# TurakhiaLab/DIPPER

Measured on AMD Instinct MI355X. Metric: tips/sec FASTA->Newick at N=30000, higher is better.
Workload: dtype f64

## Files before the change

### dipper_amd/capi.py

```python
import ctypes as C
import os

import numpy as np

_HERE = os.path.dirname(os.path.abspath(__file__))
_LIB = None

SRC_MSA, SRC_MASH, SRC_MATRIX = 1, 2, 3
DIST_UNCORRECTED, DIST_JC = 1, 2
DIST_POISSON, DIST_KIMURA = 7, 8
DIST_TN93, DIST_LOGDET, DIST_PARALINEAR = 9, 10, 11

c_i32p = C.POINTER(C.c_int32)
c_i64p = C.POINTER(C.c_int64)
c_u64p = C.POINTER(C.c_uint64)
c_f64p = C.POINTER(C.c_double)


class DipperError(RuntimeError):
    def __init__(self, code, msg):
        super().__init__(f"dipper_hip error {code}: {msg}")
        self.code = code


def library_path():
    return os.environ.get("DPR_LIB") or os.path.join(_HERE, "libdipper_hip.so")


def load_library():
    global _LIB
    if _LIB is not None:
        return _LIB
    path = library_path()
    if not os.path.exists(path):
        raise FileNotFoundError(f"{path} not built: run `python -c 'import __graft_entry__ as g; g.build()'`")
    L = C.CDLL(path)
    L.dpr_last_error.restype = C.c_char_p
    L.dpr_abi_version.restype = C.c_int
    L.dpr_pack4.argtypes = [C.c_char_p, C.c_uint64, c_u64p]
    L.dpr_pack2.argtypes = [C.c_char_p, C.c_uint64, c_u64p]
    L.dpr_pack_aa.argtypes = [C.c_char_p, C.c_uint64, C.POINTER(C.c_uint8)]
    L.dpr_njr_owner.argtypes = [C.c_int64, C.c_int]
    L.dpr_njr_local_row.argtypes = [C.c_int64, C.c_int]
    L.dpr_njr_local_row.restype = C.c_int64
    L.dpr_njr_global_pos.argtypes = [C.c_int64, C.c_int, C.c_int]
    L.dpr_njr_global_pos.restype = C.c_int64
    L.dpr_njr_rows_cap.argtypes = [C.c_int64, C.c_int]
    L.dpr_njr_rows_cap.restype = C.c_int64
    L.dpr_shard_owner.argtypes = [C.c_int64, C.c_int]
    L.dpr_shard_local_row.argtypes = [C.c_int64, C.c_int]
    L.dpr_shard_local_row.restype = C.c_int64
    L.dpr_shard_rows.argtypes = [C.c_int64, C.c_int, C.c_int]
    L.dpr_shard_rows.restype = C.c_int64
    L.dpr_shard_global_row.argtypes = [C.c_int64, C.c_int, C.c_int]
    L.dpr_shard_global_row.restype = C.c_int64
    L.dpr_record_reduce.argtypes = [C.c_void_p, C.c_int]
    L.dpr_nj_key.argtypes = [C.c_int64, C.c_int64, C.c_int64]
    L.dpr_nj_key.restype = C.c_uint64
    L.dpr_create.argtypes = [C.POINTER(C.c_void_p), C.c_int]
    L.dpr_create_virtual.argtypes = [C.POINTER(C.c_void_p), C.c_int, C.c_int]
    L.dpr_destroy.argtypes = [C.c_void_p]
    L.dpr_device_name.argtypes = [C.c_void_p, C.c_char_p, C.c_int]
    L.dpr_comm_unique_id.argtypes = [C.c_void_p]
    L.dpr_comm_init.argtypes = [C.c_void_p, C.c_int, C.c_int, C.c_void_p]
    L.dpr_comm_selftest.argtypes = [C.c_void_p]
    L.dpr_comm_info.argtypes = [C.c_void_p, C.POINTER(C.c_int), C.POINTER(C.c_int)]
    L.dpr_comm_init_local.argtypes = [C.c_void_p, C.c_int, C.c_int]
    L.dpr_comm_init_shared.argtypes = [C.c_void_p, C.c_int, C.c_int, C.c_void_p, C.c_uint64, C.c_int]
    L.dpr_comm_stats.argtypes = [C.c_void_p, C.POINTER(C.c_int), C.POINTER(C.c_int64)]
    L.dpr_shared_abort.argtypes = [C.c_void_p]
    L.dpr_shared_failed.argtypes = [C.c_void_p]
    L.dpr_shared_barrier.argtypes = [C.c_void_p, C.c_int, C.POINTER(C.c_uint32), C.c_int]
    L.dpr_shared_gather.argtypes = [C.c_void_p, C.c_int, C.c_int, C.POINTER(C.c_uint32), C.c_int, C.c_void_p, C.c_void_p, C.c_int]
    L.dpr_peer_export.argtypes = [C.c_void_p, C.c_int64, C.c_void_p]
    L.dpr_peer_attach.argtypes = [C.c_void_p, C.c_void_p]
    L.dpr_ctx_set_nj_exchange.argtypes = [C.c_void_p, C.c_int]
    L.dpr_get_nj_exchange_info.argtypes = [C.c_void_p, C.POINTER(C.c_int), C.POINTER(C.c_int64), C.POINTER(C.c_int64), C.c_char_p, C.c_int]
    L.dpr_ctx_set_poll_limit_ms.argtypes = [C.c_void_p, C.c_int]
    L.dpr_ctx_set_nj_adaptive.argtypes = [C.c_void_p, C.c_int]
    L.dpr_get_nj_adaptive_stats.argtypes = [C.c_void_p, C.POINTER(C.c_int64), C.POINTER(C.c_int64)]
    L.dpr_scan_tune.argtypes = [C.c_int, C.c_int, C.c_int]
    L.dpr_set_nj_mode.argtypes = [C.c_int]
    L.dpr_set_nj_multi_plan.argtypes = [C.c_int]
    L.dpr_nj_is_unit_sharded.argtypes = [C.c_void_p]
    L.dpr_get_nj_multi_info.argtypes = [C.c_void_p, C.c_char_p, C.c_int]
    L.dpr_ctx_set_nj_mode.argtypes = [C.c_void_p, C.c_int]
    L.dpr_ctx_set_nj_multi_plan.argtypes = [C.c_void_p, C.c_int]
    L.dpr_ctx_set_nj_virtual_shards.argtypes = [C.c_void_p, C.c_int]
    L.dpr_ctx_set_nj_kernel_timing.argtypes = [C.c_void_p, C.c_int]
    L.dpr_ctx_set_nj_variant.argtypes = [C.c_void_p, C.c_int]
    L.dpr_get_nj_lambda.argtypes = [C.c_void_p, c_f64p, C.POINTER(C.c_int64)]
    L.dpr_nj_variant_host.argtypes = [C.c_int, c_f64p, C.c_int64, C.c_int64, c_i32p, c_i32p, c_f64p, c_f64p, c_f64p, c_f64p]
    L.dpr_nj_variant_host.restype = C.c_int64
    L.dpr_get_nj_kernel_timing.argtypes = [C.c_void_p, C.POINTER(C.c_int), c_f64p, C.POINTER(C.c_int64)]
    L.dpr_nj_kernel_name.argtypes = [C.c_int]
    L.dpr_nj_kernel_name.restype = C.c_char_p
    L.dpr_get_place_timing.argtypes = [C.c_void_p, c_f64p, c_f64p]
    L.dpr_get_place_overlap.argtypes = [C.c_void_p, C.POINTER(C.c_int), c_f64p]
    L.dpr_get_place_policy.argtypes = [C.c_void_p, C.POINTER(C.c_int64), C.POINTER(C.c_int64)]
    L.dpr_get_prune_stats.argtypes = [C.c_void_p, c_u64p, c_u64p]
    L.dpr_ctx_set_debug_fault.argtypes = [C.c_void_p, C.c_int64, C.c_int]
    L.dpr_get_nj_progress.argtypes = [C.c_void_p, C.POINTER(C.c_int64), C.POINTER(C.c_int64)]
    L.dpr_get_njp_shape.argtypes = [C.c_void_p, C.POINTER(C.c_int64), C.POINTER(C.c_int), C.POINTER(C.c_int), C.POINTER(C.c_int), C.POINTER(C.c_int)]
    L.dpr_bw_probe.argtypes = [C.c_void_p, C.c_int64, C.c_int, C.c_int, C.c_int, C.POINTER(C.c_float)]
    L.dpr_set_msa.argtypes = [C.c_void_p, c_u64p, C.c_int64, C.c_int64]
    L.dpr_set_msa_aa.argtypes = [C.c_void_p, C.POINTER(C.c_uint8), C.c_int64, C.c_int64]
    L.dpr_set_reads.argtypes = [C.c_void_p, c_u64p, c_u64p, c_u64p, C.c_int64]
    L.dpr_set_matrix_lower.argtypes = [C.c_void_p, c_f64p, C.c_int64]
    L.dpr_sketch.argtypes = [C.c_void_p, C.c_int, C.c_int, c_u64p]
    L.dpr_get_mash_index_info.argtypes = [C.c_void_p, c_i64p]
    L.dpr_dist_matrix.argtypes = [C.c_void_p, C.c_int, C.c_int, C.c_int]
    L.dpr_reserve_nj.argtypes = [C.c_void_p, C.c_int64]
    L.dpr_warm_graphs.argtypes = [C.c_void_p]
    L.dpr_nj_run.argtypes = [C.c_void_p, C.c_int64, c_i32p, c_i32p, c_f64p, c_f64p, c_f64p]
    L.dpr_nj_run.restype = C.c_int64
    L.dpr_argmin_once.argtypes = [C.c_void_p, C.c_int, c_i32p, c_i32p, c_f64p, C.POINTER(C.c_float)]
    L.dpr_n_active.argtypes = [C.c_void_p]
    L.dpr_n_active.restype = C.c_int64
    L.dpr_n_total.argtypes = [C.c_void_p]
    L.dpr_n_total.restype = C.c_int64
    L.dpr_get_matrix_row.argtypes = [C.c_void_p, C.c_int64, c_f64p]
    L.dpr_get_row_sums.argtypes = [C.c_void_p, c_f64p]
    L.dpr_get_msa_counts.argtypes = [C.c_void_p, C.c_int64, c_i32p, c_i32p]
    L.dpr_msa_dist_block.argtypes = [C.c_void_p, C.c_int64, C.c_int64, C.c_int64, C.c_int, C.c_int, c_f64p, C.c_int, C.POINTER(C.c_float)]
    L.dpr_get_kmer_hashes.argtypes = [C.c_void_p, C.c_int64, C.c_int, c_u64p, c_u64p, c_u64p]
    L.dpr_get_place_state.argtypes = [C.c_void_p, c_i32p, c_f64p, c_f64p]
    L.dpr_get_place_walks.argtypes = [C.c_void_p, c_i32p, C.POINTER(C.c_int64)]
    L.dpr_get_timing.argtypes = [C.c_void_p, c_f64p, c_f64p]
    L.dpr_place_run.argtypes = [C.c_void_p, C.c_int, C.c_int, C.c_int, C.c_int64, C.c_int64,
                                c_i32p, c_i32p, c_i32p, c_i32p, c_f64p]
    L.dpr_place_exact_run.argtypes = [C.c_void_p, C.c_int, C.c_int, C.c_int, C.c_int64,
                                      c_i32p, c_i32p, c_i32p, c_i32p, c_f64p]
    L.dpr_get_exact_state.argtypes = [C.c_void_p, c_i32p, c_i32p]
    L.dpr_dc_run.argtypes = [C.c_void_p, C.c_int, C.c_int, C.c_int, C.c_int64, C.c_int64, C.c_int,
                             c_i32p, c_i32p, c_i32p, c_i32p, c_f64p, c_i32p]
    L.dpr_place_fixed_set.argtypes = [C.c_void_p, C.c_int64, C.c_int64, c_i32p, c_i32p, c_i32p, c_i32p, c_f64p]
    L.dpr_place_fixed_run.argtypes = [C.c_void_p, C.c_int, C.c_int, C.c_int, c_i32p, c_f64p, c_f64p]
    L.dpr_ctx_set_place_fixed_batch.argtypes = [C.c_void_p, C.c_int64]
    L.dpr_get_place_fixed_timing.argtypes = [C.c_void_p, c_f64p, c_f64p]
    L.dpr_njp_unit_owner.argtypes = [C.c_int64, C.c_int64, C.c_int64, C.c_int]
    L.dpr_place_policy_run.argtypes = [C.c_int, C.c_int, C.c_int, C.c_int, C.c_int64, C.c_int64, C.c_int64, C.c_int64, c_f64p, c_f64p, C.c_int64, c_i32p]
    L.dpr_nj_plan_resolve.argtypes = [C.c_int, C.c_int, C.c_int, C.c_int, C.c_int, C.c_int, C.c_int64, C.c_uint64]
    L.dpr_dc_query_share.argtypes = [C.c_int64, C.c_int64, C.c_int, C.c_int, C.POINTER(C.c_int64), C.POINTER(C.c_int64)]
    L.dpr_dc_deal_clusters.argtypes = [C.POINTER(C.c_int64), C.c_int64, C.c_int, c_i32p]
    L.dpr_get_dc_stats.argtypes = [C.c_void_p, C.POINTER(C.c_int64), c_f64p]
    L.dpr_get_dc_table_stats.argtypes = [C.c_void_p, c_i64p]
    L.dpr_msa_resample.argtypes = [C.c_void_p, C.c_uint64, C.c_int64]
    L.dpr_get_msa_boot_weights.argtypes = [C.c_void_p, c_i32p]
    L.dpr_msa_boot_weights.argtypes = [C.c_uint64, C.c_int64, C.c_int64, c_i32p]
    L.dpr_get_msa_site_coverage.argtypes = [C.c_void_p, c_i32p]
    L.dpr_msa_filter_sites.argtypes = [C.c_void_p, C.c_int]
    L.dpr_msa_filter_sites.restype = C.c_int64
    L.dpr_split_support.argtypes = [C.c_int64, c_i32p, c_i32p, c_i32p, c_i32p, c_i32p]
    L.dpr_comm_sum_i32.argtypes = [C.c_void_p, c_i32p, C.c_int64]
    L.dpr_transfer_support.argtypes = [C.c_void_p, C.c_int64, c_i32p, c_i32p, c_i32p, c_i32p, c_i64p]
    _bme_out = [C.c_int, c_i32p, c_i32p, c_f64p, c_f64p, c_i64p]
    L.dpr_bme_nni.argtypes = [C.c_void_p, C.c_int64, c_i32p, c_i32p] + _bme_out
    L.dpr_bme_nni_host.argtypes = [c_f64p, C.c_int64, c_i32p, c_i32p] + _bme_out
    L.dpr_bme_eval_host.argtypes = [c_f64p, C.c_int64, c_i32p, C.c_int32, c_f64p, c_f64p, c_i32p, c_f64p]
    L.dpr_get_bme_timing.argtypes = [C.c_void_p, c_f64p, c_f64p]
    L.dpr_get_bme_stats.argtypes = [C.c_void_p, c_i64p]
    L.dpr_bme_spr.argtypes = [C.c_void_p, C.c_int64, c_i32p, c_i32p] + _bme_out
    L.dpr_bme_spr_host.argtypes = [c_f64p, C.c_int64, c_i32p, c_i32p] + _bme_out
    L.dpr_bme_spr_eval_host.argtypes = [c_f64p, C.c_int64, c_i32p, C.c_int32, c_f64p, c_i32p, c_i32p, c_f64p]
    L.dpr_bme_spr_gain_host.argtypes = [c_f64p, C.c_int64, c_i32p, C.c_int32, C.c_int64, C.c_int32, c_f64p, c_i32p]
    L.dpr_get_bme_spr_timing.argtypes = [C.c_void_p, c_f64p]
    L.dpr_get_bme_spr_stats.argtypes = [C.c_void_p, c_i64p]
    L.dpr_upgma_run.argtypes = [C.c_void_p, C.c_int, c_i32p, c_i32p, c_f64p]
    L.dpr_upgma_run.restype = C.c_int64
    L.dpr_upgma_host.argtypes = [c_f64p, C.c_int64, C.c_int, c_i32p, c_i32p, c_f64p]
    L.dpr_get_upgma_stats.argtypes = [C.c_void_p, c_i64p]
    L.dpr_get_upgma_timing.argtypes = [C.c_void_p, c_f64p]
    L.dpr_transfer_support_host.argtypes = [C.c_int64, c_i32p, c_i32p, c_i32p, c_i32p, c_i64p]
    L.dpr_transfer_taxa.argtypes = [C.c_void_p, C.c_int64, c_i32p, c_i32p, c_i32p, c_i32p, C.c_int, c_i64p, c_i64p, c_i64p]
    L.dpr_transfer_taxa_host.argtypes = [C.c_int64, c_i32p, c_i32p, c_i32p, c_i32p, C.c_int, c_i64p, c_i64p, c_i64p]
    L.dpr_ctx_set_tbe_lds.argtypes = [C.c_void_p, C.c_int64]
    L.dpr_comm_sum_i64.argtypes = [C.c_void_p, c_i64p, C.c_int64]
    _LIB = L
    return L


DC_EXACT_LAST = 1
COMM_SHARED_BYTES = 65536
TRANSPORT_AUTO, TRANSPORT_RCCL, TRANSPORT_IPC = 0, 1, 2


class SharedRegion:

    def __init__(self, name, create=False):
        import mmap
        self.path = os.path.join("/dev/shm", name)
        if create:
            with open(self.path, "wb") as f:
                f.write(b"\0" * COMM_SHARED_BYTES)
        self._f = open(self.path, "r+b")
        self._m = mmap.mmap(self._f.fileno(), COMM_SHARED_BYTES)
        self._buf = (C.c_char * COMM_SHARED_BYTES).from_buffer(self._m)
        self.address = C.addressof(self._buf)
        self.size = COMM_SHARED_BYTES

    def abort(self):
        load_library().dpr_shared_abort(self.address)

    def failed(self):
        return bool(load_library().dpr_shared_failed(self.address))

    def barrier(self, world, sense, timeout_ms=10000):
        L = load_library()
        _chk(L, L.dpr_shared_barrier(self.address, world, C.byref(sense), timeout_ms))

    def gather(self, rank, world, sense, mine: bytes, timeout_ms=10000):
        L = load_library()
        out = (C.c_char * (len(mine) * world))()
        _chk(L, L.dpr_shared_gather(self.address, rank, world, C.byref(sense), timeout_ms, mine, out, len(mine)))
        return [bytes(out[r * len(mine):(r + 1) * len(mine)]) for r in range(world)]

    def unlink(self):
        try:
            os.unlink(self.path)
        except OSError:
            pass


def dc_virtual_ranks(w):
    return (w & 0xff) << 8


def set_nj_virtual_shards(w):
    L = load_library()
    _chk(L, L.dpr_set_nj_virtual_shards(w))


def set_nj_mode(mode):
    L = load_library()
    _chk(L, L.dpr_set_nj_mode(mode))


def set_nj_multi_plan(plan):
    L = load_library()
    _chk(L, L.dpr_set_nj_multi_plan(plan))


def _chk(L, rc):
    if rc < 0:
        raise DipperError(rc, (L.dpr_last_error() or b"").decode())
    return rc


(NJ_PLAN_SINGLE_STREAM, NJ_PLAN_SINGLE_PRUNED, NJ_PLAN_BIONJ, NJ_PLAN_ROWS_STREAM, NJ_PLAN_REPLICAS, NJ_PLAN_UNIT_SHARDED,
 NJ_PLAN_ROWS_PRUNED) = range(7)


def nj_plan_resolve(world, virtual_ranks, variant, pruned, multi_plan, virtual_shards, n, total_bytes):
    L = load_library()
    return _chk(L, L.dpr_nj_plan_resolve(world, int(virtual_ranks), variant, int(pruned), multi_plan, virtual_shards, n, total_bytes))


def place_policy_run(source, world, window_transport, no_overlap, multi_min, first, last, batch_rows, tree_ms, dist_alone_ms):
    L = load_library()
    tree = np.ascontiguousarray(tree_ms, dtype=np.float64)
    dist = np.ascontiguousarray(dist_alone_ms, dtype=np.float64)
    assert tree.shape == dist.shape and tree.ndim == 1
    beside = np.zeros(max(len(tree), 1), dtype=np.int32)
    _chk(L, L.dpr_place_policy_run(source, world, int(window_transport), int(no_overlap), multi_min, first, last, batch_rows,
                                   _p(tree, c_f64p), _p(dist, c_f64p), len(tree), _p(beside, c_i32p)))
    return [bool(b) for b in beside[:len(tree)]]


def _p(a, t):
    return a.ctypes.data_as(t)


def pack4(seq: bytes):
    L = load_library()
    out = np.zeros((len(seq) + 15) // 16, dtype=np.uint64)
    _chk(L, L.dpr_pack4(seq, len(seq), _p(out, c_u64p)))
    return out


def pack2(seq: bytes):
    L = load_library()
    out = np.zeros((len(seq) + 31) // 32, dtype=np.uint64)
    _chk(L, L.dpr_pack2(seq, len(seq), _p(out, c_u64p)))
    return out


def pack_aa(seq: bytes):
    L = load_library()
    out = np.zeros(len(seq), dtype=np.uint8)
    _chk(L, L.dpr_pack_aa(seq, len(seq), _p(out, C.POINTER(C.c_uint8))))
    return out


def pack_aa_many(seqs):
    Ls = len(seqs[0])
    out = np.full((len(seqs), Ls), 255, dtype=np.uint8)
    for i, s in enumerate(seqs):
        c = pack_aa(s)
        out[i, : min(Ls, len(c))] = c[:Ls]
    return out


def msa_boot_weights(seed, replicate, L):
    lib = load_library()
    out = np.zeros(L, dtype=np.int32)
    _chk(lib, lib.dpr_msa_boot_weights(seed, replicate, L, _p(out, c_i32p)))
    return out


def split_support(n, main_x, main_y, rep_x, rep_y, counts=None):
    lib = load_library()
    k = max(n - 2, 1)
    mx, my, rx, ry = (np.ascontiguousarray(np.asarray(a, dtype=np.int32)[: n - 2]) for a in (main_x, main_y, rep_x, rep_y))
    if counts is None:
        counts = np.zeros(k, dtype=np.int32)
    assert counts.dtype == np.int32 and counts.flags.c_contiguous and len(counts) >= n - 2
    _chk(lib, lib.dpr_split_support(n, _p(mx, c_i32p), _p(my, c_i32p), _p(rx, c_i32p), _p(ry, c_i32p), _p(counts, c_i32p)))
    return counts


def _tbe_args(n, main_x, main_y, rep_x, rep_y, phi_sum):
    logs = [np.ascontiguousarray(np.asarray(a, dtype=np.int32)[: n - 2]) for a in (main_x, main_y, rep_x, rep_y)]
    if phi_sum is None:
        phi_sum = np.zeros(max(n - 2, 1), dtype=np.int64)
    assert phi_sum.dtype == np.int64 and phi_sum.flags.c_contiguous and len(phi_sum) >= n - 2
    return logs, phi_sum


def transfer_support_host(n, main_x, main_y, rep_x, rep_y, phi_sum=None):
    lib = load_library()
    (mx, my, rx, ry), phi_sum = _tbe_args(n, main_x, main_y, rep_x, rep_y, phi_sum)
    _chk(lib, lib.dpr_transfer_support_host(n, _p(mx, c_i32p), _p(my, c_i32p), _p(rx, c_i32p), _p(ry, c_i32p), _p(phi_sum, c_i64p)))
    return phi_sum


def _taxa_args(n, moved, pairs):
    if moved is None:
        moved = np.zeros(max(n, 1), dtype=np.int64)
    if pairs is None:
        pairs = np.zeros(1, dtype=np.int64)
    assert moved.dtype == np.int64 and moved.flags.c_contiguous and len(moved) >= n
    assert pairs.dtype == np.int64 and pairs.flags.c_contiguous and len(pairs) >= 1
    return moved, pairs


def transfer_taxa_host(n, main_x, main_y, rep_x, rep_y, cutoff_permille=300, phi_sum=None, moved=None, pairs=None):
    lib = load_library()
    (mx, my, rx, ry), phi_sum = _tbe_args(n, main_x, main_y, rep_x, rep_y, phi_sum)
    moved, pairs = _taxa_args(n, moved, pairs)
    _chk(lib, lib.dpr_transfer_taxa_host(n, _p(mx, c_i32p), _p(my, c_i32p), _p(rx, c_i32p), _p(ry, c_i32p), cutoff_permille,
                                         _p(phi_sum, c_i64p), _p(moved, c_i64p), _p(pairs, c_i64p)))
    return phi_sum, moved, pairs


def _bme_args(n, merge_x, merge_y, max_rounds, nstats=4):
    mx, my = (np.ascontiguousarray(np.asarray(a, dtype=np.int32)[: max(n - 2, 0)]) for a in (merge_x, merge_y))
    assert len(mx) == len(my) == n - 2
    out = dict(kids=np.zeros(2 * max(n - 2, 1), dtype=np.int32), top=np.zeros(1, dtype=np.int32), len=np.zeros(2 * n - 2, dtype=np.float64),
               L_rounds=np.zeros(max_rounds + 1, dtype=np.float64), stats=np.zeros(nstats, dtype=np.int64))
    ptrs = (_p(mx, c_i32p), _p(my, c_i32p), max_rounds, _p(out["kids"], c_i32p), _p(out["top"], c_i32p), _p(out["len"], c_f64p),
            _p(out["L_rounds"], c_f64p), _p(out["stats"], c_i64p))
    return (mx, my), out, ptrs


def _bme_result(n, out):
    rounds, moves, fallbacks, cands0 = (int(v) for v in out["stats"][:4])
    more = dict(long_moves=int(out["stats"][4]), max_k=int(out["stats"][5])) if len(out["stats"]) == 6 else {}
    return dict(**more, kids=out["kids"][: 2 * (n - 2)].reshape(n - 2, 2), top=int(out["top"][0]), len=out["len"], L_rounds=out["L_rounds"][: rounds + 1],
                rounds=rounds, moves=moves, fallbacks=fallbacks, candidates0=cands0)


def bme_nni_host(D, merge_x, merge_y, max_rounds):
    lib = load_library()
    D = np.asarray(D, dtype=np.float64)
    n = D.shape[0]
    rows = np.ascontiguousarray(np.concatenate([D[i, :i] for i in range(n)])) if n > 1 else np.zeros(1)
    keep, out, ptrs = _bme_args(n, merge_x, merge_y, max_rounds)
    _chk(lib, lib.dpr_bme_nni_host(_p(rows, c_f64p), n, *ptrs))
    return _bme_result(n, out)


def bme_eval_host(D, kids, top):
    lib = load_library()
    D = np.asarray(D, dtype=np.float64)
    n = D.shape[0]
    rows = np.ascontiguousarray(np.concatenate([D[i, :i] for i in range(n)]))
    kids = np.ascontiguousarray(np.asarray(kids, dtype=np.int32).reshape(-1))
    assert len(kids) == 2 * (n - 2)
    ln, gain, move = np.zeros(2 * n - 2), np.zeros(2 * n - 2), np.zeros(2 * n - 2, dtype=np.int32)
    L = C.c_double(0.0)
    _chk(lib, lib.dpr_bme_eval_host(_p(rows, c_f64p), n, _p(kids, c_i32p), int(top), _p(ln, c_f64p), _p(gain, c_f64p), _p(move, c_i32p), C.byref(L)))
    return dict(len=ln, gain=gain, move=move, L=L.value)


def _lower_rows(D):
    D = np.asarray(D, dtype=np.float64)
    n = D.shape[0]
    return n, (np.ascontiguousarray(np.concatenate([D[i, :i] for i in range(n)])) if n > 1 else np.zeros(1))


def bme_spr_host(D, merge_x, merge_y, max_rounds):
    lib = load_library()
    n, rows = _lower_rows(D)
    keep, out, ptrs = _bme_args(n, merge_x, merge_y, max_rounds, 6)
    _chk(lib, lib.dpr_bme_spr_host(_p(rows, c_f64p), n, *ptrs))
    return _bme_result(n, out)


def bme_spr_eval_host(D, kids, top):
    lib = load_library()
    n, rows = _lower_rows(D)
    kids = np.ascontiguousarray(np.asarray(kids, dtype=np.int32).reshape(-1))
    assert len(kids) == 2 * (n - 2)
    m2 = 2 * (2 * n - 2)
    gain, w, k = np.zeros(m2), np.zeros(m2, dtype=np.int32), np.zeros(m2, dtype=np.int32)
    L = C.c_double(0.0)
    _chk(lib, lib.dpr_bme_spr_eval_host(_p(rows, c_f64p), n, _p(kids, c_i32p), int(top), _p(gain, c_f64p), _p(w, c_i32p), _p(k, c_i32p), C.byref(L)))
    return dict(gain=gain, w=w, k=k, L=L.value)


def bme_spr_gain_host(D, kids, top, d, w):
    lib = load_library()
    n, rows = _lower_rows(D)
    kids = np.ascontiguousarray(np.asarray(kids, dtype=np.int32).reshape(-1))
    assert len(kids) == 2 * (n - 2)
    g, k = C.c_double(0.0), C.c_int32(0)
    _chk(lib, lib.dpr_bme_spr_gain_host(_p(rows, c_f64p), n, _p(kids, c_i32p), int(top), int(d), int(w), C.byref(g), C.byref(k)))
    return g.value, k.value


NJ_VARIANT_NJ, NJ_VARIANT_BIONJ = 0, 1


def upgma_host(D, linkage=0):
    lib = load_library()
    n, rows = _lower_rows(D)
    cnt = max(n - 1, 1)
    mx, my, h = np.zeros(cnt, dtype=np.int32), np.zeros(cnt, dtype=np.int32), np.zeros(cnt, dtype=np.float64)
    _chk(lib, lib.dpr_upgma_host(_p(rows, c_f64p), n, int(linkage), _p(mx, c_i32p), _p(my, c_i32p), _p(h, c_f64p)))
    return dict(merge_x=mx[: n - 1], merge_y=my[: n - 1], height=h[: n - 1])


def nj_variant_host(variant, D, max_iters=-1):
    lib = load_library()
    D = np.asarray(D, dtype=np.float64)
    n = D.shape[0]
    rows = np.ascontiguousarray(np.concatenate([D[i, :i] for i in range(n)])) if n > 1 else np.zeros(1)
    k = max(n - 2, 1)
    mx = np.zeros(k, dtype=np.int32)
    my = np.zeros(k, dtype=np.int32)
    bx = np.zeros(k, dtype=np.float64)
    by = np.zeros(k, dtype=np.float64)
    lam = np.full(k, 0.5, dtype=np.float64)
    last = C.c_double(0.0)
    done = _chk(lib, lib.dpr_nj_variant_host(variant, _p(rows, c_f64p), n, max_iters, _p(mx, c_i32p), _p(my, c_i32p), _p(bx, c_f64p),
                                             _p(by, c_f64p), C.byref(last), _p(lam, c_f64p)))
    return dict(iters=done, merge_x=mx[:done], merge_y=my[:done], bl_x=bx[:done], bl_y=by[:done], last_d=last.value, lam=lam[:done])


def pack4_many(seqs):
    Ls = len(seqs[0])
    W = (Ls + 15) // 16
    out = np.zeros((len(seqs), W), dtype=np.uint64)
    for i, s in enumerate(seqs):
        w = pack4(s)
        out[i, : min(W, len(w))] = w[:W]
    return out


class Dipper:

    def __init__(self, device=0, virtual_world=0):
        self.L = load_library()
        h = C.c_void_p()
        if virtual_world:
            _chk(self.L, self.L.dpr_create_virtual(C.byref(h), device, virtual_world))
        else:
            _chk(self.L, self.L.dpr_create(C.byref(h), device))
        self.h = h

    def close(self):
        if self.h:
            self.L.dpr_destroy(self.h)
            self.h = None

    def __del__(self):
        try:
            self.close()
        except Exception:
            pass

    def device_name(self):
        buf = C.create_string_buffer(256)
        _chk(self.L, self.L.dpr_device_name(self.h, buf, 256))
        return buf.value.decode()

    def comm_unique_id(self):
        buf = (C.c_char * 128)()
        _chk(self.L, self.L.dpr_comm_unique_id(buf))
        return bytes(buf)

    def comm_init(self, rank, world, uid: bytes):
        buf = (C.c_char * 128).from_buffer_copy(uid) if uid else None
        _chk(self.L, self.L.dpr_comm_init(self.h, rank, world, buf))

    def comm_selftest(self):
        _chk(self.L, self.L.dpr_comm_selftest(self.h))

    def comm_init_local(self, rank, world):
        _chk(self.L, self.L.dpr_comm_init_local(self.h, rank, world))

    def comm_init_shared(self, rank, world, region, transport=0):
        self._region = region
        _chk(self.L, self.L.dpr_comm_init_shared(self.h, rank, world, region.address, region.size, transport))

    def comm_stats(self):
        t = C.c_int()
        n = C.c_int64()
        _chk(self.L, self.L.dpr_comm_stats(self.h, C.byref(t), C.byref(n)))
        return ["none", "rccl", "ipc", "local"][t.value], int(n.value)

    def peer_export(self, n_tips):
        buf = (C.c_char * 192)()
        _chk(self.L, self.L.dpr_peer_export(self.h, n_tips, buf))
        return bytes(buf)

    def peer_attach(self, blobs):
        data = b"".join(blobs)
        buf = (C.c_char * len(data)).from_buffer_copy(data)
        _chk(self.L, self.L.dpr_peer_attach(self.h, buf))

    def set_nj_exchange(self, plan):
        _chk(self.L, self.L.dpr_ctx_set_nj_exchange(self.h, plan))

    def nj_exchange_info(self):
        p = C.c_int()
        nl = C.c_int64()
        nc = C.c_int64()
        note = C.create_string_buffer(256)
        _chk(self.L, self.L.dpr_get_nj_exchange_info(self.h, C.byref(p), C.byref(nl), C.byref(nc), note, 256))
        return {"plan": {0: "legacy", 1: "peer", 2: "mailbox"}.get(p.value, str(p.value)), "launches": int(nl.value),
                "collectives": int(nc.value), "note": note.value.decode()}

    def set_nj_adaptive(self, on):
        _chk(self.L, self.L.dpr_ctx_set_nj_adaptive(self.h, on))

    def nj_adaptive_stats(self):
        a = C.c_int64()
        b = C.c_int64()
        _chk(self.L, self.L.dpr_get_nj_adaptive_stats(self.h, C.byref(a), C.byref(b)))
        return int(a.value), int(b.value)

    def set_debug_fault(self, iteration, rank):
        _chk(self.L, self.L.dpr_ctx_set_debug_fault(self.h, iteration, rank))

    def set_poll_limit_ms(self, ms):
        _chk(self.L, self.L.dpr_ctx_set_poll_limit_ms(self.h, ms))

    def comm_info(self):
        r = C.c_int()
        n = C.c_int()
        _chk(self.L, self.L.dpr_comm_info(self.h, C.byref(r), C.byref(n)))
        return r.value, n.value

    def set_msa(self, packed4, L):
        p = np.ascontiguousarray(packed4, dtype=np.uint64)
        _chk(self.L, self.L.dpr_set_msa(self.h, _p(p, c_u64p), p.shape[0], L))
        self._msa_sites = int(L)

    def set_msa_aa(self, codes):
        p = np.ascontiguousarray(codes, dtype=np.uint8)
        assert p.ndim == 2
        _chk(self.L, self.L.dpr_set_msa_aa(self.h, _p(p, C.POINTER(C.c_uint8)), p.shape[0], p.shape[1]))
        self._msa_sites = int(p.shape[1])

    def set_matrix_lower(self, rows, n):
        r = np.ascontiguousarray(rows, dtype=np.float64)
        assert r.size == n * (n - 1) // 2
        _chk(self.L, self.L.dpr_set_matrix_lower(self.h, _p(r, c_f64p), n))

    def set_matrix_full(self, D):
        D = np.asarray(D, dtype=np.float64)
        n = D.shape[0]
        rows = np.concatenate([D[i, :i] for i in range(n)]) if n > 1 else np.zeros(0)
        self.set_matrix_lower(rows, n)

    def set_reads(self, seqs):
        words = [pack2(s) for s in seqs]
        lens = np.array([len(s) for s in seqs], dtype=np.uint64)
        nw = np.array([len(w) for w in words], dtype=np.uint64)
        off = np.zeros(len(seqs), dtype=np.uint64)
        off[1:] = np.cumsum(nw)[:-1]
        flat = np.concatenate(words) if len(words) else np.zeros(0, np.uint64)
        if flat.size == 0:
            flat = np.zeros(1, np.uint64)
        self._reads = (np.ascontiguousarray(flat), off, lens)
        _chk(self.L, self.L.dpr_set_reads(self.h, _p(self._reads[0], c_u64p), _p(off, c_u64p), _p(lens, c_u64p), len(seqs)))

    def set_reads_packed(self, flat, off, lens):
        flat = np.ascontiguousarray(flat, dtype=np.uint64)
        off = np.ascontiguousarray(off, dtype=np.uint64)
        lens = np.ascontiguousarray(lens, dtype=np.uint64)
        self._reads = (flat, off, lens)
        _chk(self.L, self.L.dpr_set_reads(self.h, _p(flat, c_u64p), _p(off, c_u64p), _p(lens, c_u64p), len(lens)))

    def sketch(self, k=15, S=1000, fetch=True):
        n = len(self._reads[2])
        out = np.zeros((n, S), dtype=np.uint64) if fetch else None
        _chk(self.L, self.L.dpr_sketch(self.h, k, S, _p(out, c_u64p) if fetch else None))
        return out

    def mash_index_info(self):
        info = np.zeros(8, dtype=np.int64)
        _chk(self.L, self.L.dpr_get_mash_index_info(self.h, _p(info, c_i64p)))
        names = ("built", "chunk_tips", "chunks", "distinct", "dense", "dense_min", "max_sketch", "beside_task_bound")
        return {nm: int(v) for nm, v in zip(names, info)}

    def kmer_hashes(self, seq, k):
        _, off, lens = self._reads
        nk = max(int(lens[seq]) - k + 1, 0)
        out = np.zeros(max(nk, 1), dtype=np.uint64)
        _chk(self.L, self.L.dpr_get_kmer_hashes(self.h, seq, k, _p(off, c_u64p), _p(lens, c_u64p), _p(out, c_u64p)))
        return out[:nk]

    def place_run(self, source, n, first=2, dist_type=1, k=15, state=None):
        st = state or dict(head=np.full(2 * n, -1, np.int32), e=np.full(8 * n, -1, np.int32),
                           nxt=np.full(8 * n, -1, np.int32), belong=np.full(8 * n, -1, np.int32),
                           len=np.full(8 * n, 2.0, np.float64))
        _chk(self.L, self.L.dpr_place_run(self.h, source, dist_type, k, first, n, _p(st["head"], c_i32p),
                                          _p(st["e"], c_i32p), _p(st["nxt"], c_i32p), _p(st["belong"], c_i32p),
                                          _p(st["len"], c_f64p)))
        cid = np.zeros(40 * n, np.int32)
        cdis = np.zeros(40 * n, np.float64)
        trace = np.zeros(3 * n, np.float64)
        _chk(self.L, self.L.dpr_get_place_state(self.h, _p(cid, c_i32p), _p(cdis, c_f64p), _p(trace, c_f64p)))
        st.update(cid=cid, cdis=cdis, trace=trace.reshape(n, 3))
        return st

    def place_exact_run(self, source, n, dist_type=1, k=15):
        st = dict(head=np.full(2 * n, -1, np.int32), e=np.full(8 * n, -1, np.int32),
                  nxt=np.full(8 * n, -1, np.int32), belong=np.full(8 * n, -1, np.int32),
                  len=np.full(8 * n, 2.0, np.float64))
        _chk(self.L, self.L.dpr_place_exact_run(self.h, source, dist_type, k, n, _p(st["head"], c_i32p),
                                                _p(st["e"], c_i32p), _p(st["nxt"], c_i32p),
                                                _p(st["belong"], c_i32p), _p(st["len"], c_f64p)))
        rev = np.zeros(8 * n, np.int32)
        dep = np.zeros(2 * n, np.int32)
        trace = np.zeros(3 * n, np.float64)
        _chk(self.L, self.L.dpr_get_exact_state(self.h, _p(rev, c_i32p), _p(dep, c_i32p)))
        _chk(self.L, self.L.dpr_get_place_state(self.h, None, None, _p(trace, c_f64p)))
        st.update(rev=rev, dep=dep, trace=trace.reshape(n, 3))
        return st

    def dc_run(self, source, n, backbone, dist_type=1, k=15, flags=0):
        st = dict(head=np.full(2 * n, -1, np.int32), e=np.full(8 * n, -1, np.int32),
                  nxt=np.full(8 * n, -1, np.int32), belong=np.full(8 * n, -1, np.int32),
                  len=np.full(8 * n, 2.0, np.float64))
        cl = np.full(n, -1, np.int32)
        _chk(self.L, self.L.dpr_dc_run(self.h, source, dist_type, k, n, backbone, flags, _p(st["head"], c_i32p),
                                       _p(st["e"], c_i32p), _p(st["nxt"], c_i32p), _p(st["belong"], c_i32p),
                                       _p(st["len"], c_f64p), _p(cl, c_i32p)))
        cid = np.zeros(40 * n, np.int32)
        cdis = np.zeros(40 * n, np.float64)
        trace = np.zeros(3 * n, np.float64)
        _chk(self.L, self.L.dpr_get_place_state(self.h, _p(cid, c_i32p), _p(cdis, c_f64p), _p(trace, c_f64p)))
        counts = np.zeros(5, np.int64)
        ms = np.zeros(3, np.float64)
        _chk(self.L, self.L.dpr_get_dc_stats(self.h, counts.ctypes.data_as(C.POINTER(C.c_int64)), _p(ms, c_f64p)))
        st.update(cid=cid, cdis=cdis, trace=trace.reshape(n, 3), cluster_id=cl,
                  stats=dict(clusters=int(counts[0]), max_cluster=int(counts[1]), pairs=int(counts[2]),
                             groups=int(counts[3]), jobs=int(counts[4]), backbone_ms=float(ms[0]),
                             assign_ms=float(ms[1]), cluster_ms=float(ms[2])))
        return st

    def dc_table_stats(self):
        out = np.zeros(4, dtype=np.int64)
        _chk(self.L, self.L.dpr_get_dc_table_stats(self.h, _p(out, c_i64p)))
        return {nm: int(v) for nm, v in zip(("entries", "chunks", "max_entries", "max_leaves"), out)}

    def place_fixed_set(self, m, n, state):
        st = {k: np.ascontiguousarray(state[k], dtype=np.float64 if k == "len" else np.int32) for k in ("head", "e", "nxt", "belong", "len")}
        assert st["head"].size >= 2 * n and all(st[k].size >= 8 * n for k in ("e", "nxt", "belong", "len"))
        _chk(self.L, self.L.dpr_place_fixed_set(self.h, m, n, _p(st["head"], c_i32p), _p(st["e"], c_i32p), _p(st["nxt"], c_i32p),
                                                _p(st["belong"], c_i32p), _p(st["len"], c_f64p)))
        self._pfix_nq = n - m

    def place_fixed_run(self, source, dist_type=1, k=15):
        nq = max(getattr(self, "_pfix_nq", 1), 1)
        slot = np.full(nq, -2, np.int32)
        frac = np.zeros(nq, np.float64)
        add = np.zeros(nq, np.float64)
        _chk(self.L, self.L.dpr_place_fixed_run(self.h, source, dist_type, k, _p(slot, c_i32p), _p(frac, c_f64p), _p(add, c_f64p)))
        return slot, frac, add

    def set_place_fixed_batch(self, queries):
        _chk(self.L, self.L.dpr_ctx_set_place_fixed_batch(self.h, queries))

    def place_fixed_timing(self):
        a = C.c_double()
        b = C.c_double()
        _chk(self.L, self.L.dpr_get_place_fixed_timing(self.h, C.byref(a), C.byref(b)))
        return a.value, b.value

    def warm_graphs(self):
# ... 274 lines not shown
```

### dipper_amd/csrc/ctx_nj.hip

```cpp
#include "ctx_internal.hpp"

#include <chrono>
#include <cstdio>

namespace dpr {
static int g_nj_mode = -1;
static int g_nj_vshards = 1;
static int g_nj_multi_plan = -1;
constexpr int64_t kNjShardTips = 65536;
static int nj_multi_plan()
{
    if (g_nj_multi_plan < 0) {
        const char* e = std::getenv("DPR_NJ_MULTI");
        g_nj_multi_plan = (e && std::strcmp(e, "shard") == 0) ? 1 : (e && std::strcmp(e, "solo") == 0) ? 2 : (e && std::strcmp(e, "rows") == 0) ? 3 : 0;
    }
    return g_nj_multi_plan;
}

bool want_pruned(const dpr_ctx* c)
{
    if (c->nj_mode >= 0) return c->nj_mode == 1;
    if (g_nj_mode < 0) {
        const char* e = std::getenv("DPR_NJ_MODE");
        g_nj_mode = (e && std::strcmp(e, "stream") == 0) ? 0 : 1;
// ... 101 lines not shown
    if (!c->plan.rows_dealt()) return DPR_OK;
    if (int rc = njs_setup(c, njr)) return rc;
    if (njr && c->plan.exchange == kNjsLegacy) {
        set_error("dpr_dist_matrix: the row-sharded pruned NJ needs the peers' buffers mapped on every rank (" + c->nj_exchange_note + "); use DPR_NJ_MODE=stream");
        return DPR_ERR_STATE;
    }
    return DPR_OK;
}
static int dist_fill(dpr_ctx* c, int source, int dist_type, int64_t n)
{
    for (auto& b : c->nj) {
        if (source == DPR_SRC_MSA) {
            if (int rc = msa_dist_rows(c->msa, b, dist_type, c->stream)) return rc;
        } else if (source == DPR_SRC_MASH) {
            if (b.world > 1) {
                if (int rc = mash_dist_matrix_sharded(c->mash, b.rank, b.world, b.rows_local, b.D, b.ld, c->stream)) return rc;
            } else {
                for (int64_t r0 = 0; r0 < b.rows_local; r0 += 32768) {
                    const int64_t nr = b.rows_local - r0 < 32768 ? b.rows_local - r0 : 32768;
                    if (int rc = mash_dist_rows(c->mash, r0, nr, b.rank, b.world, true, n, b.D + r0 * b.ld, b.ld, c->stream)) return rc;
                }
            }
        } else {
            if (int rc = nj_expand_lower(b, c->packed_lower, c->stream)) return rc;
        }
        if (c->plan.kind == DPR_NJ_PLAN_BIONJ)
            if (int rc = nj_bionj_init(b, c->stream)) return rc;
    }
    return DPR_OK;
}
static int dist_row_sums(dpr_ctx* c)
{
    const bool dealt = c->plan.rows_dealt(), windows = dealt && c->plan.exchange != kNjsLegacy;
    for (auto& b : c->nj)
        if (int rc = nj_init_sums(b, c->stream, !dealt ? nullptr : windows ? reinterpret_cast<double*>(b.peer.win + b.peer.lay.off_slice) : b.slice)) return rc;
    if (dealt)
        if (int rc = windows ? njs_barrier(c) : exchange(c, EX_U)) return rc;
    for (auto& b : c->nj) {
        if (dealt)
            if (int rc = windows ? njs_launch_unpack_u(b, c->stream) : nj_launch_unpack_u(b, c->stream)) return rc;
        if (int rc = nj_prepare(b, c->stream)) return rc;
    }
    return DPR_OK;
}
static int dist_build_njr(dpr_ctx* c)
{
    int rplan = c->nj_exchange == 2 ? kNjrMailbox : c->nj_exchange == 1 ? kNjrCollective : (c->local_comm ? kNjrMailbox : kNjrCollective);
    if (c->nj_exchange < 0 && !c->local_comm)
        if (const char* e = std::getenv("DPR_NJ_EXCHANGE")) rplan = std::strcmp(e, "mailbox") == 0 ? kNjrMailbox : kNjrCollective;
    if (rplan == kNjrCollective && c->vworld == 0 && !comm_real(c)) { set_error("dpr_dist_matrix: the collective plan of the row-sharded pruned NJ needs a transport between the ranks (RCCL, or dpr_comm_init_shared)"); return DPR_ERR_STATE; }
    for (auto& b : c->nj) {
        b.rs.world = c->world; b.rs.rank = b.rank; b.rs.plan = rplan;
        b.rs.win_off = b.peer.lay.off_njr;
        b.rs.gather = njr_gather_cb; b.rs.cb_ctx = c;
        b.rs.barrier = (c->vworld == 0 && (c->comm || (c->shm && rplan == kNjrCollective))) ? njr_barrier_cb : nullptr;
        b.rs.launches = 0; b.rs.collectives = 0;
    }
    std::vector<NjBuffers*> ranks = njr_ranks(c);
    if (int rc = njr_build(ranks, c->stream)) return rc;
    c->nj_exchange_note = std::string("row-sharded pruned NJ (njr.hip), exchange plan ") + (rplan == kNjrMailbox ? "mailbox" : "collective");
    return DPR_OK;
}
static void njp_set_shards(dpr_ctx* c, int kind)
{
    NjPruned& q = c->nj[0].pr;
    if (kind == DPR_NJ_PLAN_UNIT_SHARDED) { q.sh_world = c->world; q.sh_rank = c->rank; q.sh_virtual = false; q.gather = njp_gather_cb; q.gather_ctx = c; }
    else if (ctx_vshards(c) > 1) { q.sh_world = ctx_vshards(c); q.sh_rank = 0; q.sh_virtual = true; }
}
static int dist_build_njp(dpr_ctx* c)
{
    NjPruned& q = c->nj[0].pr;
    njp_set_shards(c, c->plan.kind);
    if (c->nj_adaptive >= 0) q.adaptive = c->nj_adaptive;
    if (int rc = njp_build(c->nj[0], c->stream)) return rc;
    if (c->nj_adaptive >= 0) q.adaptive = c->nj_adaptive;
    return DPR_OK;
}
static bool plan_is_njp(int kind) { return kind == DPR_NJ_PLAN_SINGLE_PRUNED || kind == DPR_NJ_PLAN_REPLICAS || kind == DPR_NJ_PLAN_UNIT_SHARDED; }

}

using namespace dpr;

__global__ void dpr_warm_kernel(int x);

extern "C" {

int dpr_dist_matrix(dpr_ctx* c, int source, int dist_type, int k)
{
    if (!c) { set_error("dpr_dist_matrix: null ctx"); return DPR_ERR_ARG; }
    DPR_HIP(hipSetDevice(c->device));
    if (c->world > 1 && c->vworld == 0 && !c->comm && !c->local_comm && !c->shm) { set_error("dpr_dist_matrix: dpr_comm_init was not called"); return DPR_ERR_STATE; }
    int64_t n = 0;
    if (source == DPR_SRC_MSA) {
        if (!c->msa.planes) { set_error("dpr_dist_matrix: call dpr_set_msa first"); return DPR_ERR_STATE; }
        n = c->msa.n;
    } else if (source == DPR_SRC_MATRIX) {
        if (!c->packed_lower) { set_error("dpr_dist_matrix: call dpr_set_matrix_lower first"); return DPR_ERR_STATE; }
        n = c->n_input;
    } else if (source == DPR_SRC_MASH) {
        if (!c->mash.sketches) { set_error("dpr_dist_matrix: call dpr_set_reads and dpr_sketch first"); return DPR_ERR_STATE; }
        if (k != c->mash.k) { set_error("dpr_dist_matrix: k differs from the sketch k"); return DPR_ERR_ARG; }
        n = c->mash.n;
    } else {
        set_error("dpr_dist_matrix: source not available");
        return DPR_ERR_ARG;
    }
    const int kind = ctx_nj_plan(c, n, "dpr_dist_matrix");
    if (kind < 0) return kind;
    c->have_matrix = 0;
    c->plan = NjPlan{ kind, kNjsLegacy };
    c->nj_exchange_note.clear();
    if (int rc = dist_alloc(c, n)) return rc;
    DPR_HIP(hipEventRecord(c->ev[0], c->stream));
    if (int rc = dist_fill(c, source, dist_type, n)) return rc;
    if (int rc = dist_row_sums(c)) return rc;
    if (int rc = kind == DPR_NJ_PLAN_ROWS_PRUNED ? dist_build_njr(c) : plan_is_njp(kind) ? dist_build_njp(c) : DPR_OK) return rc;
    DPR_HIP(hipEventRecord(c->ev[1], c->stream));
    DPR_HIP(hipStreamSynchronize(c->stream));
    float ms = 0;
    DPR_HIP(hipEventElapsedTime(&ms, c->ev[0], c->ev[1]));
    c->dist_ms = ms;
    c->have_matrix = 1;
    return DPR_OK;
}

int dpr_reserve_nj(dpr_ctx* c, int64_t n)
{
    if (!c || n < 2 || n >= (1 << 24)) { set_error("dpr_reserve_nj: bad argument"); return DPR_ERR_ARG; }
    DPR_HIP(hipSetDevice(c->device));
    const int kind = ctx_nj_plan(c, n, "dpr_reserve_nj");
    if (kind < 0) return kind;
    if (kind != DPR_NJ_PLAN_SINGLE_STREAM && kind != DPR_NJ_PLAN_SINGLE_PRUNED && kind != DPR_NJ_PLAN_BIONJ) return DPR_OK;
    c->have_matrix = 0;
    if (int rc = nj_alloc(c->nj[0], n, 0, 1, c->stream, 0, kind == DPR_NJ_PLAN_BIONJ)) return rc;
    if (kind == DPR_NJ_PLAN_SINGLE_PRUNED) {
        njp_set_shards(c, kind);
        if (int rc = njp_arena(c->nj[0].pr, n, c->stream)) return rc;
    }
    DPR_HIP(hipStreamSynchronize(c->stream));
    return DPR_OK;
}

int dpr_warm_graphs(dpr_ctx* c)
{
    if (!c) { set_error("dpr_warm_graphs: null ctx"); return DPR_ERR_ARG; }
    DPR_HIP(hipSetDevice(c->device));
    const bool tlog = log_level("cli") > 0;
    const auto t0 = std::chrono::steady_clock::now();
    auto lap = [&](const char* what) {
        if (tlog) std::fprintf(stderr, "  dpr_warm_graphs: %s at %.1f ms\n", what, std::chrono::duration<double, std::milli>(std::chrono::steady_clock::now() - t0).count());
    };
    hipStream_t st = c->stream;
    if (hipStreamBeginCapture(st, hipStreamCaptureModeThreadLocal) == hipSuccess) {
        hipLaunchKernelGGL(dpr_warm_kernel, dim3(1), dim3(64), 0, st, 0);
        ScopedGraph g;
        ScopedGraphExec ge;
        if (hipStreamEndCapture(st, g.put()) == hipSuccess && g) {
            if (hipGraphInstantiate(ge.put(), g, nullptr, nullptr, 0) == hipSuccess && ge) {
                lap("first hipGraphInstantiate");
                (void)hipGraphLaunch(ge, st);
                (void)hipStreamSynchronize(st);
                lap("graph replayed");
            }
        }
    }
    {
        DevBuf<char> d;
        constexpr size_t kWarmBytes = 512 << 10;
        if (d.alloc(kWarmBytes) == hipSuccess) {
            std::vector<char> h(kWarmBytes);
            (void)hipMemsetAsync(d, 0, kWarmBytes, st);
            (void)hipStreamSynchronize(st);
            (void)hipMemcpyAsync(h.data(), d, kWarmBytes, hipMemcpyDeviceToHost, st);
            (void)hipStreamSynchronize(st);
            (void)hipMemcpyAsync(d, h.data(), kWarmBytes, hipMemcpyHostToDevice, st);
            (void)hipStreamSynchronize(st);
        }
    }
    lap("staged copies both ways");
    (void)hipGetLastError();
    return DPR_OK;
}

}
namespace dpr {
int fetch_state(dpr_ctx* c, NjState* st)
{
    DPR_HIP(hipMemcpyAsync(st, c->nj[0].st, sizeof(NjState), hipMemcpyDeviceToHost, c->stream));
    DPR_HIP(hipStreamSynchronize(c->stream));
    return DPR_OK;
}
}
extern "C" {

int64_t dpr_nj_run(dpr_ctx* c, int64_t max_iters, int32_t* merge_x, int32_t* merge_y, double* bl_x,
                   double* bl_y, double* last_d)
{
    if (!c || !c->have_matrix) { set_error("dpr_nj_run: call dpr_dist_matrix first"); return DPR_ERR_STATE; }
    DPR_HIP(hipSetDevice(c->device));
    NjState st;
    if (int rc = fetch_state(c, &st)) return rc;
    int64_t todo = st.n - 2;
    if (todo < 0) todo = 0;
    if (max_iters >= 0 && max_iters < todo) todo = max_iters;
    const int64_t it0 = st.it;
    c->nj[0].kt = &c->nj_kt;
    if (c->nj_kt.stride > 0 && it0 == 0) { c->nj_kt.samples = 0; for (double& v : c->nj_kt.us_sum) v = 0; }
    c->nj_launches = 0; c->nj_collectives = 0;
    DPR_HIP(hipEventRecord(c->ev[2], c->stream));
    if (c->plan.kind == DPR_NJ_PLAN_ROWS_PRUNED) {
        std::vector<NjBuffers*> ranks = njr_ranks(c);
        c->nj[0].rs.launches = 0; c->nj[0].rs.collectives = 0;
        if (int rc = njr_run(ranks, it0, todo, c->stream)) return rc;
        c->nj_launches = c->nj[0].rs.launches; c->nj_collectives = c->nj[0].rs.collectives;
    } else if (plan_is_njp(c->plan.kind)) {
        if (int rc = njp_run(c->nj[0], it0, todo, c->stream)) return rc;
    } else {
        for (int64_t k = 0; k < todo; ++k)
            if (int rc = nj_iteration(c, st.n - k, it0 + k)) return rc;
    }
    DPR_HIP(hipEventRecord(c->ev[3], c->stream));
    if (c->plan.one_exchange_loop()) {
        if (int rc = njs_barrier(c)) return rc;
        for (auto& b : c->nj)
            if (int rc = njs_launch_finish(b, st.n - todo, it0 + todo, c->njs_pending, c->stream)) return rc;
        c->njs_pending = false;
        if (int rc = njs_barrier(c)) return rc;
    } else {
        for (auto& b : c->nj)
            if (!b.pr.active)
                if (int rc = nj_launch_finish(b, st.n - todo, it0 + todo, c->stream)) return rc;
    }
    if (int rc = fetch_state(c, &st)) return rc;
    float ms = 0;
    DPR_HIP(hipEventElapsedTime(&ms, c->ev[2], c->ev[3]));
    c->nj_ms = ms;
    if (!c->nj_kt.ev.empty()) {
        NjKernelTiming& kt = c->nj_kt;
        const size_t grp = (size_t)kt.nk + 1;
        for (size_t g0 = 0; kt.nk > 0 && g0 + grp <= kt.ev.size(); g0 += grp) {
            for (int k = 0; k < kt.nk; ++k) {
                float us = 0;
                if (hipEventElapsedTime(&us, kt.ev[g0 + (size_t)k], kt.ev[g0 + (size_t)k + 1]) == hipSuccess) kt.us_sum[k] += (double)us * 1e3;
            }
            ++kt.samples;
        }
        for (hipEvent_t e : kt.ev) (void)hipEventDestroy(e);
        kt.ev.clear();
    }
    const int64_t done = st.it - it0;
    if (done > 0) {
        if (merge_x) DPR_HIP(hipMemcpy(merge_x, c->nj[0].log_x + it0, sizeof(int32_t) * (size_t)done, hipMemcpyDeviceToHost));
        if (merge_y) DPR_HIP(hipMemcpy(merge_y, c->nj[0].log_y + it0, sizeof(int32_t) * (size_t)done, hipMemcpyDeviceToHost));
        if (bl_x) DPR_HIP(hipMemcpy(bl_x, c->nj[0].log_bx + it0, sizeof(double) * (size_t)done, hipMemcpyDeviceToHost));
        if (bl_y) DPR_HIP(hipMemcpy(bl_y, c->nj[0].log_by + it0, sizeof(double) * (size_t)done, hipMemcpyDeviceToHost));
    }
    if (st.status == 3) {
        set_error("dpr_nj_run: the exchange between the ranks failed (a rank's record did not arrive within the poll limit, or the all-gather delivered a stale one)");
        return DPR_ERR_COMM;
    }
    if (st.status == 4) {
        char msg[320];
        std::snprintf(msg, sizeof msg, "dpr_nj_run: the ranks' replicated row sums differ after %lld iterations (rank %d: %a, rank %d: %a): a row pulled from its owner "
                      "was stale or torn -- the merge log up to here is not trustworthy; use the legacy exchange (dpr_ctx_set_nj_exchange(ctx, 0))",
                      (long long)st.it, (int)st.x, st.q, (int)st.y, st.d);
        set_error(msg);
        return DPR_ERR_COMM;
    }
    if (st.status == 5) {
        set_error("dpr_nj_run: internal: the test blocks of the post kernel did not see the producer blocks' tag within 2 ms (njp_post2_kernel; DPR_NJP_POST2=0 selects the fused kernel)");
        return DPR_ERR_HIP;
    }
    if (st.status != 0) {
        set_error("dpr_nj_run: no Q candidate below the reference's init value 10000 (undefined in the reference)");
        return DPR_ERR_NOCAND;
    }
    if (last_d && st.n == 2) {
        NjBuffers& b0 = c->nj[0];
        int32_t pos01[2] = { 0, 1 };
        if (b0.pr.in_positions()) DPR_HIP(hipMemcpy(pos01, b0.pr.pos_of_slot, sizeof(pos01), hipMemcpyDeviceToHost));
        const double* row1 = slot_row(c, 1, pos01[1], true);
        const bool by_record = c->plan.rows_dealt() && c->vworld == 0 && c->plan.exchange == kNjsLegacy;
        if (row1 && !by_record) {
            DPR_HIP(hipMemcpy(last_d, row1 + pos01[0], sizeof(double), hipMemcpyDeviceToHost));
        } else {
            NjRecord rec{ 0.0, 0ull, 0.0, 0ull };
            if (row1) DPR_HIP(hipMemcpy(&rec.d, row1 + pos01[0], sizeof(double), hipMemcpyDeviceToHost));
            DPR_HIP(hipMemcpy(b0.recs + c->rank, &rec, sizeof(NjRecord), hipMemcpyHostToDevice));
            if (int rc = exchange(c, EX_RECS)) return rc;
            DPR_HIP(hipStreamSynchronize(c->stream));
            DPR_HIP(hipMemcpy(&rec, b0.recs + 0, sizeof(NjRecord), hipMemcpyDeviceToHost));
            *last_d = rec.d;
        }
    }
    return done;
}

int dpr_argmin_once(dpr_ctx* c, int reps, int32_t* out_i, int32_t* out_j, double* out_q, float* out_ms)
{
    if (!c || !c->have_matrix) { set_error("dpr_argmin_once: call dpr_dist_matrix first"); return DPR_ERR_STATE; }
    DPR_HIP(hipSetDevice(c->device));
    if (reps < 1) reps = 1;
    NjState st0;
    if (int rc = fetch_state(c, &st0)) return rc;
    auto probe = [&](NjBuffers& b) -> int {
        return b.pr.in_positions() ? nj_launch_scan(b, true, b.pr.P, 0, c->stream) : nj_launch_scan(b, true, st0.n, st0.it, c->stream);
    };
    for (auto& b : c->nj)
        if (int rc = probe(b)) return rc;
    DPR_HIP(hipEventRecord(c->ev[2], c->stream));
    for (int r = 0; r < reps; ++r)
        for (auto& b : c->nj)
            if (int rc = probe(b)) return rc;
    DPR_HIP(hipEventRecord(c->ev[3], c->stream));
    for (auto& b : c->nj)
        if (int rc = nj_launch_select_local(b, nj_scan_grid(), c->stream)) return rc;
    if (int rc = exchange(c, EX_RECS)) return rc;
    const int ew = c->plan.whole_matrix() ? 1 : c->world;
    std::vector<NjRecord> recs((size_t)ew);
    DPR_HIP(hipMemcpyAsync(recs.data(), c->nj[0].recs, sizeof(NjRecord) * (size_t)ew, hipMemcpyDeviceToHost, c->stream));
    DPR_HIP(hipStreamSynchronize(c->stream));
    float ms = 0;
    DPR_HIP(hipEventElapsedTime(&ms, c->ev[2], c->ev[3]));
    if (out_ms) *out_ms = ms / (float)reps;
    const int w = dpr_record_reduce(recs.data(), ew);
    if (w < 0 || !(recs[(size_t)w].q < 10000.0)) { set_error("dpr_argmin_once: no Q candidate below 10000"); return DPR_ERR_NOCAND; }
    const NjRecord& rec = recs[(size_t)w];
    if (out_i) *out_i = (int32_t)(rec.key & 0xFFFFFFull);
    if (out_j) *out_j = (int32_t)((rec.key >> 24) & 0xFFFFFFull);
    if (out_q) *out_q = rec.q;
    return DPR_OK;
}

int dpr_nj_plan_resolve(int world, int virtual_ranks, int variant, int pruned, int multi_plan, int virtual_shards, int64_t n, uint64_t total_bytes)
{
    if (world < 1 || variant < 0 || variant > 1 || multi_plan < 0 || multi_plan > 3 || virtual_shards < 1 || n < 2) { set_error("dpr_nj_plan_resolve: bad argument"); return DPR_ERR_ARG; }
    if (variant == 1) {
        if (!virtual_ranks && virtual_shards == 1) return DPR_NJ_PLAN_BIONJ;
        set_error("BIONJ runs the single-rank streaming plan: not on a context of virtual ranks or with virtual shards (dpr_set_nj_virtual_shards > 1)");
        return DPR_ERR_ARG;
    }
    if (!pruned || n < 3) return world > 1 ? DPR_NJ_PLAN_ROWS_STREAM : DPR_NJ_PLAN_SINGLE_STREAM;
    if (world == 1) return DPR_NJ_PLAN_SINGLE_PRUNED;
    if (multi_plan == 3) return DPR_NJ_PLAN_ROWS_PRUNED;
    if (virtual_ranks) return DPR_NJ_PLAN_ROWS_STREAM;
    if (multi_plan == 0 && 2.0 * 8.0 * (double)n * (double)n > 0.85 * (double)total_bytes) return DPR_NJ_PLAN_ROWS_PRUNED;
    return multi_plan == 1 || (multi_plan == 0 && n >= kNjShardTips) ? DPR_NJ_PLAN_UNIT_SHARDED : DPR_NJ_PLAN_REPLICAS;
}

int dpr_njp_unit_owner(int64_t strip, int64_t group, int64_t P, int world) { return njp_unit_owner(strip, group, P, world); }

int dpr_set_nj_virtual_shards(int w)
{
    if (w < 1 || w > 64) { set_error("dpr_set_nj_virtual_shards: 1 <= w <= 64"); return DPR_ERR_ARG; }
    g_nj_vshards = w;
    return DPR_OK;
}

int dpr_set_nj_multi_plan(int plan)
{
    if (plan < 0 || plan > 3) { set_error("dpr_set_nj_multi_plan: 0 auto, 1 unit-sharded, 2 single-GPU plan on every rank, 3 row-sharded pruned"); return DPR_ERR_ARG; }
    g_nj_multi_plan = plan;
    return DPR_OK;
}
int dpr_nj_is_unit_sharded(dpr_ctx* c) { return c && c->plan.kind == DPR_NJ_PLAN_UNIT_SHARDED ? 1 : 0; }
int dpr_get_nj_multi_info(dpr_ctx* c, char* buf, int cap)
{
    if (!c || !buf || cap <= 0) { set_error("dpr_get_nj_multi_info: bad argument"); return DPR_ERR_ARG; }
    static const char* const ex[] = { "legacy (two all-gathers per iteration)", "peer (one all-gather, rows pulled)", "mailbox (no collective)" };
    std::string s = "single rank";
    switch (c->plan.kind) {
    case DPR_NJ_PLAN_BIONJ: if (c->world > 1) s = "BIONJ, streaming, every rank its own copy"; break;
    case DPR_NJ_PLAN_ROWS_PRUNED: s = c->nj_exchange_note; break;
    case DPR_NJ_PLAN_UNIT_SHARDED: s = "pruned, matrix replicated, unit tests and scans sharded (one all-gather of block records per iteration)"; break;
    case DPR_NJ_PLAN_REPLICAS: s = "pruned, every rank runs the single-GPU plan on its own copy of the matrix (replicas)"; break;
    case DPR_NJ_PLAN_ROWS_STREAM: s = std::string("streaming, rows sharded block-cyclically, exchange ") + ex[c->plan.exchange >= 0 && c->plan.exchange <= 2 ? c->plan.exchange : 0]; break;
    }
    std::snprintf(buf, (size_t)cap, "%s", s.c_str());
    return DPR_OK;
}

int dpr_ctx_set_nj_mode(dpr_ctx* c, int mode)
{
    if (!c || mode < -1 || mode > 1) { set_error("dpr_ctx_set_nj_mode: mode must be -1, 0 or 1"); return DPR_ERR_ARG; }
    c->nj_mode = mode;
    return DPR_OK;
}
int dpr_ctx_set_nj_multi_plan(dpr_ctx* c, int plan)
{
    if (!c || plan < -1 || plan > 3) { set_error("dpr_ctx_set_nj_multi_plan: -1 default, 0 auto, 1 unit-sharded, 2 single-GPU plan on every rank, 3 row-sharded pruned"); return DPR_ERR_ARG; }
    c->nj_multi_plan = plan;
    return DPR_OK;
}
int dpr_ctx_set_nj_variant(dpr_ctx* c, int variant)
{
    if (!c || variant < 0 || variant > 1) { set_error("dpr_ctx_set_nj_variant: variant must be 0 (NJ) or 1 (BIONJ)"); return DPR_ERR_ARG; }
    c->nj_variant = variant;
    return DPR_OK;
}
int dpr_get_nj_lambda(dpr_ctx* c, double* out, int64_t* count)
{
    if (!c || !count) { set_error("dpr_get_nj_lambda: null argument"); return DPR_ERR_ARG; }
    if (!c->have_matrix || c->plan.kind != DPR_NJ_PLAN_BIONJ || !c->nj[0].log_lam) { set_error("dpr_get_nj_lambda: no BIONJ matrix (dpr_ctx_set_nj_variant(ctx, 1), then dpr_dist_matrix)"); return DPR_ERR_STATE; }
    DPR_HIP(hipSetDevice(c->device));
    NjState st;
    if (int rc = fetch_state(c, &st)) return rc;
    *count = st.it;
    if (out && st.it > 0) DPR_HIP(hipMemcpy(out, c->nj[0].log_lam, sizeof(double) * (size_t)st.it, hipMemcpyDeviceToHost));
    return DPR_OK;
}
int dpr_ctx_set_nj_kernel_timing(dpr_ctx* c, int stride)
{
    if (!c || stride < 0) { set_error("dpr_ctx_set_nj_kernel_timing: stride >= 0"); return DPR_ERR_ARG; }
    c->nj_kt.stride = stride;
    return DPR_OK;
}
int dpr_get_nj_kernel_timing(dpr_ctx* c, int* kernels, double* us_avg, int64_t* samples)
{
    if (!c) { set_error("dpr_get_nj_kernel_timing: null ctx"); return DPR_ERR_ARG; }
    if (kernels) *kernels = c->nj_kt.nk;
    if (samples) *samples = c->nj_kt.samples;
    if (us_avg) for (int k = 0; k < kNjKernelsMax; ++k) us_avg[k] = c->nj_kt.samples > 0 ? c->nj_kt.us_sum[k] / (double)c->nj_kt.samples : 0.0;
    return DPR_OK;
}
const char* dpr_nj_kernel_name(int idx) { return njp_kernel_name(idx); }
int dpr_get_nj_phase_stamps(uint64_t* out) { return njp_phase_stamps((unsigned long long*)out); }
int dpr_get_njp_list(dpr_ctx* c, int32_t* out, int64_t cap, int64_t* count, int64_t* positions, double* ur, int64_t ur_cap)
{
    if (!c || !out || !count || !positions) { set_error("dpr_get_njp_list: null argument"); return DPR_ERR_ARG; }
    DPR_HIP(hipSetDevice(c->device));
    return njp_debug_list(c->nj[0], out, cap, count, positions, ur, ur_cap);
}

int dpr_ctx_set_nj_virtual_shards(dpr_ctx* c, int w)
{
    if (!c || w < -1 || w == 0 || w > 64) { set_error("dpr_ctx_set_nj_virtual_shards: -1 or 1 <= w <= 64"); return DPR_ERR_ARG; }
    c->nj_vshards = w;
    return DPR_OK;
}

int dpr_set_nj_mode(int mode)
{
    if (mode != 0 && mode != 1) { set_error("dpr_set_nj_mode: mode must be 0 or 1"); return DPR_ERR_ARG; }
    g_nj_mode = mode;
    return DPR_OK;
}

int dpr_ctx_set_nj_adaptive(dpr_ctx* c, int on)
{
    if (!c || on < -1 || on > 1) { set_error("dpr_ctx_set_nj_adaptive: -1, 0 or 1"); return DPR_ERR_ARG; }
    c->nj_adaptive = on;
    return DPR_OK;
}
int dpr_get_nj_adaptive_stats(dpr_ctx* c, int64_t* stream_iterations, int64_t* stream_epochs)
{
    if (!c || !c->have_matrix || !c->nj[0].pr.active) { set_error("dpr_get_nj_adaptive_stats: pruned path not active"); return DPR_ERR_STATE; }
    if (stream_iterations) *stream_iterations = c->nj[0].pr.stream_iterations;
    if (stream_epochs) *stream_epochs = c->nj[0].pr.stream_epochs;
    return DPR_OK;
}

int dpr_get_prune_stats(dpr_ctx* c, uint64_t* units_scanned, uint64_t* units_per_full_scan)
{
    if (!c || !c->have_matrix || !c->nj[0].pr.active) { set_error("dpr_get_prune_stats: pruned path not active"); return DPR_ERR_STATE; }
    NjState st;
    if (int rc = fetch_state(c, &st)) return rc;
    if (units_scanned) *units_scanned = st.units_scanned;
    if (units_per_full_scan) *units_per_full_scan = (uint64_t)c->nj[0].pr.utot0;
    return DPR_OK;
}


int dpr_get_nj_progress(dpr_ctx* c, int64_t* iterations_done, int64_t* active)
{
    if (!c || !c->have_matrix) { set_error("dpr_get_nj_progress: call dpr_dist_matrix first"); return DPR_ERR_STATE; }
    DPR_HIP(hipSetDevice(c->device));
    NjState st;
    if (int rc = fetch_state(c, &st)) return rc;
    if (iterations_done) *iterations_done = st.it;
    if (active) *active = st.n;
    return DPR_OK;
}

}
namespace {
double host_tree256(double* c)
{
    for (int s = 128; s > 0; s >>= 1)
        for (int t = 0; t < s; ++t) c[t] = c[t] + c[t + s];
    return c[0];
}
double host_fold(const double* part, int64_t nchunk)
{
    double p[256];
    for (int t = 0; t < 256; ++t) {
        double acc = 0.0;
        for (int64_t c = t; c < nchunk; c += 256) acc += part[c];
        p[t] = acc;
    }
    return host_tree256(p);
}
}
extern "C" {

int64_t dpr_nj_variant_host(int variant, const double* lower_rows, int64_t N, int64_t max_iters, int32_t* merge_x, int32_t* merge_y,
                            double* bl_x, double* bl_y, double* last_d, double* lambda)
{
    if ((variant != 0 && variant != 1) || N < 2 || N >= (1 << 24) || (N > 2 && (!lower_rows || !merge_x || !merge_y || !bl_x || !bl_y))) {
        set_error("dpr_nj_variant_host: bad argument");
        return DPR_ERR_ARG;
    }
    const bool bionj = variant == 1;
    const int64_t ld = N;
    std::vector<double> D((size_t)(N * ld), 0.0), V, U((size_t)N), Ur((size_t)N), part((size_t)((N + 255) / 256 + 1));
    for (int64_t i = 0; i < N; ++i)
        for (int64_t j = 0; j < i; ++j) D[(size_t)(i * ld + j)] = D[(size_t)(j * ld + i)] = lower_rows[i * (i - 1) / 2 + j];
    if (bionj) V = D;
    for (int64_t i = 0; i < N; ++i) {
        double c[256];
        for (int t = 0; t < 256; ++t) {
            double acc = 0.0;
            for (int64_t j = t; j < N; j += 256)
                if (j != i) acc += D[(size_t)(i * ld + j)];
            c[t] = acc;
        }
        U[(size_t)i] = host_tree256(c);
    }
    int64_t it = 0;
    for (; it < N - 2; ++it) {
        if (max_iters >= 0 && it >= max_iters) break;
        const int64_t n = N - it, last = n - 1, nchunk = (n + 255) / 256;
        const double r = (double)(n - 2);
        for (int64_t i = 0; i < n; ++i) Ur[(size_t)i] = U[(size_t)i] / r;
        double bq = 10000.0;
        uint64_t bk = ~0ull;
        for (int64_t a = 1; a < n; ++a) {
            const double* row = D.data() + a * ld;
            const double ua = Ur[(size_t)a];
            for (int64_t c = 0; c < a; ++c) {
                const double dv = row[c], uc = Ur[(size_t)c];
                const double q1 = (dv - ua) - uc, q2 = (dv - uc) - ua;
                if (q1 <= bq) { const uint64_t k = dpr_nj_key(a, c, n); if (q1 < bq || k < bk) { bq = q1; bk = k; } }
                if (q2 <= bq) { const uint64_t k = dpr_nj_key(c, a, n); if (q2 < bq || k < bk) { bq = q2; bk = k; } }
            }
        }
        if (bk == ~0ull || !(bq < 10000.0)) break;
        const int64_t ki = (int64_t)(bk & 0xFFFFFFull), kj = (int64_t)((bk >> 24) & 0xFFFFFFull);
        const int64_t x = ki < kj ? ki : kj, y = ki < kj ? kj : ki;
        const double d = D[(size_t)(y * ld + x)];
        const double bx0 = (d + U[(size_t)x] / r - U[(size_t)y] / r) * 0.5, by0 = d - bx0;
        double blX = bx0, blY = by0;
        if (blX < 0) { blY += blX; blX = 0; }
        if (blY < 0) { blX += blY; blY = 0; }
        merge_x[it] = (int32_t)x; merge_y[it] = (int32_t)y; bl_x[it] = blX; bl_y[it] = blY;
        double lam = 0.5, vxy = 0.0;
        if (bionj) {
            vxy = V[(size_t)(y * ld + x)];
            for (int64_t c = 0; c < nchunk; ++c) {
                double v[256];
                for (int t = 0; t < 256; ++t) {
                    const int64_t k = c * 256 + t;
                    v[t] = (k < n && k != x && k != y) ? V[(size_t)(y * ld + k)] - V[(size_t)(x * ld + k)] : 0.0;
                }
                part[(size_t)c] = host_tree256(v);
            }
            const double ssum = host_fold(part.data(), nchunk);
            lam = 0.5 + ssum / (2.0 * r * vxy);
            if (vxy == 0.0 || lam != lam) lam = 0.5;
            else if (lam < 0.0) lam = 0.0;
            else if (lam > 1.0) lam = 1.0;
            if (lambda) lambda[it] = lam;
        }
        for (int64_t c = 0; c < nchunk; ++c) {
            double v[256];
            for (int t = 0; t < 256; ++t) {
                const int64_t i = c * 256 + t;
                double val = 0.0;
                if (i < n && i != x && i != y) {
                    const double dxi = D[(size_t)(x * ld + i)], dyi = D[(size_t)(y * ld + i)];
                    double vnew = 0.0;
                    if (bionj) {
                        const double vxi = V[(size_t)(x * ld + i)], vyi = V[(size_t)(y * ld + i)];
                        const double a = dxi - bx0, b = dyi - by0;
                        val = b + lam * (a - b);
                        vnew = vyi + lam * (vxi - vyi) - (lam * (1.0 - lam)) * vxy;
                    } else {
                        val = (dxi + dyi - d) * 0.5;
                    }
                    if (i != last) {
                        const double far = D[(size_t)(last * ld + i)];
                        U[(size_t)i] = U[(size_t)i] + (-dxi - dyi + val);
                        D[(size_t)(x * ld + i)] = val; D[(size_t)(i * ld + x)] = val;
                        D[(size_t)(y * ld + i)] = far; D[(size_t)(i * ld + y)] = far;
                        if (bionj) {
                            const double vfar = V[(size_t)(last * ld + i)];
                            V[(size_t)(x * ld + i)] = vnew; V[(size_t)(i * ld + x)] = vnew;
                            V[(size_t)(y * ld + i)] = vfar; V[(size_t)(i * ld + y)] = vfar;
                        }
                    } else {
                        U[(size_t)y] = U[(size_t)last] + (-dxi - dyi + val);
                        D[(size_t)(x * ld + y)] = val; D[(size_t)(y * ld + x)] = val;
                        if (bionj) { V[(size_t)(x * ld + y)] = vnew; V[(size_t)(y * ld + x)] = vnew; }
                    }
                }
                v[t] = val;
            }
            part[(size_t)c] = host_tree256(v);
        }
        U[(size_t)x] = host_fold(part.data(), nchunk);
    }
    if (it == N - 2 && last_d) *last_d = D[(size_t)(1 * ld + 0)];
// ... 11 lines not shown
```

### dipper_amd/csrc/dpr_internal.hpp

```cpp
#pragma once
#include <hip/hip_runtime.h>
#include <stdint.h>
#include <string>
#include <vector>

#include "../../include/dipper_hip.h"
#include "hip_scope.hpp"

namespace dpr {

constexpr int kRowBlock = DPR_ROW_BLOCK;
constexpr int kTileCols = 512;
constexpr int kScanBlocks = 8192;
constexpr int kThreads = 256;

void set_error(const std::string& msg);
int log_level(const char* category);
int hip_fail(hipError_t e, const char* what);
#define DPR_HIP(call)                                            \
    do {                                                         \
        hipError_t e__ = (call);                                 \
        if (e__ != hipSuccess) return dpr::hip_fail(e__, #call); \
    } while (0)

__host__ __device__ inline int shard_owner(int64_t row, int world)
{
    return (int)((row / kRowBlock) % world);
}
__host__ __device__ inline int64_t shard_local_row(int64_t row, int world)
{
    return (row / kRowBlock / world) * kRowBlock + row % kRowBlock;
}
__host__ __device__ inline int64_t shard_global_row(int64_t local, int rank, int world)
{
    return ((local / kRowBlock) * world + rank) * kRowBlock + local % kRowBlock;
}
__host__ __device__ inline int64_t shard_rows(int64_t n, int rank, int world)
{
    int64_t nblk = n / kRowBlock, rem = n % kRowBlock;
    int64_t full = nblk / world + ((nblk % world) > rank ? 1 : 0);
    int64_t cnt = full * kRowBlock;
    if (rem && (nblk % world) == rank) cnt += rem;
    return cnt;
}

__host__ __device__ inline uint64_t nj_band(int64_t i, int64_t n)
{
    int64_t sz0 = n / 256, rem = n % 256, thr = (sz0 + 1) * rem;
    return (uint64_t)(i < thr ? i / (sz0 + 1) : rem + (i - thr) / sz0);
}
__host__ __device__ inline uint64_t nj_key_a(int64_t i, int64_t n)
{
    return (nj_band(i, n) << 56) | (uint64_t)i;
}
__host__ __device__ inline uint64_t nj_key_b(int64_t j)
{
    return ((uint64_t)(j & 255) << 48) | ((uint64_t)j << 24);
}

__host__ __device__ inline uint64_t mix64(uint64_t z)
{
    z += 0x9E3779B97F4A7C15ull;
    z = (z ^ (z >> 30)) * 0xBF58476D1CE4E5B9ull;
    z = (z ^ (z >> 27)) * 0x94D049BB133111EBull;
    return z ^ (z >> 31);
}
__host__ __device__ inline uint64_t boot_key(uint64_t seed, int64_t replicate) { return mix64(seed ^ mix64((uint64_t)replicate)); }
__host__ __device__ inline int64_t boot_column(uint64_t key, int64_t t, int64_t L)
{
    return (int64_t)(((mix64(key ^ (uint64_t)t) >> 32) * (uint64_t)L) >> 32);
}

struct alignas(32) NjRecord {
    double q;
    uint64_t key;
    double d;
    uint64_t pad;
};

struct NjState {
    int64_t n;
    int64_t it;
    int32_t x, y;
    double d;
    double q;
    int32_t status;
    int32_t pad;
    int64_t itb;
    int64_t it_limit;
    int64_t N;
    unsigned long long cnt_list[4];
    unsigned long long units_scanned;
    int32_t pnew[2];
};

struct NjPruned {
    bool active = false;
    int64_t P = 0, ld = 0;
    double* D = nullptr;
    double* U = nullptr;
    double* Ur = nullptr;
    double* R = nullptr;
    int64_t vstride = 0;
    uint64_t *KA = nullptr, *KB = nullptr;
    bool range_known = false;
    char* t2_hdr = nullptr; double *t2_rmax = nullptr, *t2_cmax = nullptr, *t2_colmin = nullptr, *t2_rowmin = nullptr, *t2_cmin = nullptr;
    int32_t *slot_of_pos = nullptr, *pos_of_slot = nullptr, *perm = nullptr;
    uint64_t* umin = nullptr;
    int64_t nunits_alloc = 0, utot = 0;
    int64_t utot0 = 0;
    bool fresh = false;
    int sh_world = 1, sh_rank = 0;
    bool sh_virtual = false;
    int (*gather)(void* ctx, void* buf, size_t bytes_per_rank, hipStream_t s) = nullptr;
    void* gather_ctx = nullptr;
    unsigned long long* cnt_all = nullptr;
    int64_t list_stride = 0;
    double* arena_D = nullptr;
    char* arena_slab[2] = { nullptr, nullptr };
    size_t arena_slab_bytes = 0;
    int64_t arena_N = 0;
    int arena_ranks = 0;
    int epoch_index = 0;
    hipGraphExec_t graph = nullptr;
    int scan_grid = 512;
    int graph_iters = 32;
    int adaptive = 1;
    double stream_frac = 0.7;
    bool slots_mode = false;
    int64_t slots_probe_n = 0;
    int probe_fail_streak = 0;
    int64_t stream_iterations = 0, stream_epochs = 0;
    bool in_positions() const { return active && !slots_mode; }
    unsigned long long* dbg = nullptr;
    int64_t dbg_it = -1;
    int32_t* list = nullptr;
    int32_t *blk_cb = nullptr, *blk_g0 = nullptr;
    int nprep = 0;
};

constexpr int kNjKernelsMax = 6;
struct NjKernelTiming {
    int stride = 0;
    int nk = 0;
    std::vector<hipEvent_t> ev;
    double us_sum[kNjKernelsMax] = { 0, 0, 0, 0, 0, 0 };
    int64_t samples = 0;
};
inline int nj_timing_mark(NjKernelTiming* kt, bool on, hipStream_t s)
{
    if (!on) return DPR_OK;
    hipEvent_t e = nullptr;
    DPR_HIP(hipEventCreate(&e));
    kt->ev.push_back(e);
    DPR_HIP(hipEventRecord(e, s));
    return DPR_OK;
}

constexpr int kNjsMaxWorld = 64;
constexpr unsigned int kNjsTicketGroups = 32;
constexpr size_t kNjsTicketBytes = 128 * (1 + (size_t)kNjsTicketGroups);
constexpr int kNjsLegacy = 0;
constexpr int kNjsPeer = 1;
constexpr int kNjsMailbox = 2;
struct alignas(64) NjsRec {
    double q;
    uint64_t key;
    double d;
    uint64_t seq;
    uint64_t ux;
    uint64_t status;
    uint64_t pad[2];
};
struct NjsLayout {
    int64_t off_bar = 0, off_slice = 0, off_rows = 0, bytes = 0;
    int64_t off_njr = 0;
    int64_t slice_len = 0;
    int64_t ldv = 0;
};
struct NjPeer {
    int plan = kNjsLegacy;
    char* win = nullptr;
    NjsLayout lay;
    unsigned int* ticket = nullptr;
    char** d_win = nullptr;
    double** d_D = nullptr;
    std::vector<double*> h_D;
    std::vector<char*> h_win;
    std::vector<void*> opened;
    bool attached = false;
    unsigned long long bar_epoch = 0;
    unsigned long long run_id = 0;
    unsigned long long poll_ticks = 200000000ull;
    int64_t fault_it = -1; int fault_rank = -1;
};

constexpr int kNjrChunk = 1024;
constexpr int kNjrCollective = 1;
constexpr int kNjrMailbox = 2;
__host__ __device__ inline int njr_owner(int64_t p, int world) { return (int)((p / kNjrChunk) % world); }
__host__ __device__ inline int64_t njr_local_row(int64_t p, int world) { return (p / kNjrChunk / world) * kNjrChunk + p % kNjrChunk; }
__host__ __device__ inline int64_t njr_global_pos(int64_t l, int rank, int world) { return ((l / kNjrChunk) * world + rank) * kNjrChunk + l % kNjrChunk; }
__host__ __device__ inline int64_t njr_rows_cap(int64_t P, int world)
{
    const int64_t chunks = (P + kNjrChunk - 1) / kNjrChunk;
    return ((chunks + world - 1) / world) * kNjrChunk;
}
__host__ __device__ inline int64_t njr_slice_len(int64_t N, int world) { return ((N / kNjrChunk + 2 + world - 1) / world) * kNjrChunk; }
struct NjrLayout {
    int64_t off_recflag = 0, off_recs = 0, off_rowflag = 0, off_rows = 0, bytes = 0;
    int64_t rec_stride = 0;
    int64_t slice = 0;
};
struct NjRowShard {
    int world = 1, rank = 0, plan = 0;
    NjrLayout lay;
    int64_t win_off = 0;
    double* rows_plain = nullptr;
    double* stage = nullptr;
    int64_t stage_rows = 0, stage_ld = 0;
    char** d_region = nullptr;
    double** d_src = nullptr;
    unsigned int* ticket = nullptr;
    double* half[2] = { nullptr, nullptr };
    std::vector<double*> peer_half[2];
    int (*gather)(void* ctx, int kind, hipStream_t s) = nullptr;
    int (*barrier)(void* ctx) = nullptr;
    void* cb_ctx = nullptr;
    int64_t launches = 0, collectives = 0;
};

struct NjBuffers {
    NjPeer peer;
    NjKernelTiming* kt = nullptr;
    double* D = nullptr;
    int64_t twin_rows = 0;
    size_t half_bytes = 0;
    int64_t ld = 0;
    int64_t N = 0;
    int64_t rows_local = 0;
    double* U = nullptr;
    double* Ur = nullptr;
    uint64_t* KA = nullptr;
    NjRecord* partials = nullptr;
    NjRecord* recs = nullptr;
    NjsRec* recs64 = nullptr;
    double* xpart = nullptr;
    double* gath = nullptr;
    double* slice = nullptr;
    int64_t slice_len = 0;
    NjState* st = nullptr;
    int32_t* log_x = nullptr;
    int32_t* log_y = nullptr;
    double* log_bx = nullptr;
    double* log_by = nullptr;
    double* V = nullptr;
    double* vpart = nullptr;
    double* bj = nullptr;
    double* log_lam = nullptr;
    int rank = 0, world = 1;
    NjPruned pr;
    NjRowShard rs;
};

int nj_alloc(NjBuffers& b, int64_t N, int rank, int world, hipStream_t s, int64_t twin_rows = 0, bool bionj = false);
int nj_bionj_init(NjBuffers& b, hipStream_t s);
int nj_launch_bionj_lambda(NjBuffers& b, int64_t n, hipStream_t s);
int nj_launch_bionj_post(NjBuffers& b, int64_t n, int64_t it, hipStream_t s);
int nj_fill_pads(double* D, int64_t ld, int64_t nrows, int64_t ncols, int64_t rows_alloc, int64_t tail, bool diag, hipStream_t s);
void nj_free(NjBuffers& b);
int nj_expand_lower(NjBuffers& b, const double* d_packed_lower, hipStream_t s);
int nj_init_sums(NjBuffers& b, hipStream_t s, double* local_sums = nullptr);
int nj_prepare(NjBuffers& b, hipStream_t s);
int nj_launch_scan(NjBuffers& b, bool probe, int64_t n, int64_t it, hipStream_t s);
void nj_scan_config(int rg, int nt, int grid);
int nj_scan_grid();
int nj_bw_probe(const double* buf, int64_t cap_bytes, double* sink, int64_t bytes, int nt, int grid, int reps, hipStream_t s, hipEvent_t e0,
                hipEvent_t e1, float* ms);
int nj_launch_post(NjBuffers& b, int64_t n, int64_t it, hipStream_t s);
int nj_launch_select_local(NjBuffers& b, int nparts, hipStream_t s);
int nj_launch_commit_extract(NjBuffers& b, int64_t n, int64_t it, hipStream_t s);
int nj_launch_update_sharded(NjBuffers& b, int64_t n, hipStream_t s);
int nj_launch_unpack_u(NjBuffers& b, hipStream_t s);
int nj_launch_finish(NjBuffers& b, int64_t n, int64_t it, hipStream_t s);

NjsLayout njs_layout(int64_t N, int world, bool with_njr = false);
int njs_alloc_window(NjBuffers& b, hipStream_t s);
void njs_free_window(NjBuffers& b);
int njs_set_peers(NjBuffers& b, char* const* wins, double* const* Ds, hipStream_t s);
int njs_launch_scan(NjBuffers& b, int64_t n, int64_t it, bool pending, hipStream_t s);
int njs_launch_post(NjBuffers& b, int64_t n, int64_t it, bool pending, hipStream_t s);
int njs_launch_finish(NjBuffers& b, int64_t n, int64_t it, bool pending, hipStream_t s);
int njs_launch_barrier(NjBuffers& b, hipStream_t s);
int njs_launch_unpack_u(NjBuffers& b, hipStream_t s);

NjrLayout njr_layout(int64_t N, int world);
int njr_build(std::vector<NjBuffers*>& ranks, hipStream_t s);
int njr_run(std::vector<NjBuffers*>& ranks, int64_t it0, int64_t todo, hipStream_t s);
void njr_free(NjBuffers& b);

int njp_build(NjBuffers& b, hipStream_t s);
void njp_free(NjPruned& q);
int njp_arena(NjPruned& q, int64_t N, hipStream_t s);
void njp_reset(NjPruned& q);
int njp_unit_owner(int64_t strip, int64_t group, int64_t P, int world);
int njp_run(NjBuffers& b, int64_t it0, int64_t todo, hipStream_t s);
const char* njp_kernel_name(int idx);
void njp_set_kernel_names(const char* const* names);
int njp_phase_stamps(unsigned long long* out);
int njp_debug_list(NjBuffers& b, int32_t* out, int64_t cap, int64_t* count, int64_t* P, double* ur, int64_t urcap);
const double* njp_current_u(const NjPruned& q, int64_t it);
int njp_shape(const NjPruned& q, int64_t* positions, int* row_groups, int* strips, int* post2, int* scan_grid);

constexpr int kDcLeaves = 10;
struct PairJobs {
    const int4* jobs;
    const int32_t* members;
    const int32_t* cols;
    const int64_t* cl_moff;
    const int32_t* cl_m;
    const int64_t* cl_coff;
    const int64_t* cl_out;
    const int32_t* cl_ld;
    double* out;
};

struct MsaBuffers {
    uint32_t* planes = nullptr;
    int64_t n = 0, L = 0, W32 = 0;
    double* jc_tab = nullptr;
    unsigned long long* xstage = nullptr;
    uint32_t* alt_planes = nullptr;
    unsigned long long* alt_xstage = nullptr;
    int32_t* boot_w = nullptr;
    uint32_t* boot_incl = nullptr;
    int32_t* boot_src = nullptr;
    int64_t replicate = -1;
    bool aa = false;
    int32_t* aa_nx = nullptr;
};
constexpr int64_t kMsaTabSites = 1024;
constexpr int kMsaBand = 15;
int msa_upload(MsaBuffers& m, const uint64_t* packed4, int64_t n, int64_t L, hipStream_t s);
void msa_free(MsaBuffers& m);
int msa_restage(MsaBuffers& m, hipStream_t s);
int msa_derived_alloc(MsaBuffers& m);
int msa_derive(MsaBuffers& m, hipStream_t s);
int mi_inclusive_scan(const uint32_t* in, uint32_t* out, int64_t n, hipStream_t s);
int msa_dist_rows(const MsaBuffers& m, NjBuffers& b, int dist_type, hipStream_t s);
int msa_dist_tile_edge(const MsaBuffers& m, int dist_type);
int msa_counts_row(const MsaBuffers& m, int64_t row, int32_t* d_useful, int32_t* d_match, hipStream_t s);

struct TbeBuffers {
    int64_t n = 0, cap = 0;
    std::vector<int32_t> hx, hy;
    std::vector<int32_t> mpos;
    std::vector<int32_t> node;
    std::vector<int32_t> size;
    std::vector<int32_t> hphi;
    int2* main_iv = nullptr;
    int32_t* m = nullptr;
    int2* rep_iv = nullptr;
    int32_t* phi = nullptr;
    uint4* scratch = nullptr;
    size_t scratch_bytes = 0;
    int32_t skip = -1;
    int64_t taxa_cap = 0;
    int32_t* phi_arg = nullptr;
    int32_t* moved = nullptr;
    std::vector<int32_t> hmoved;
};
void tbe_free(TbeBuffers& t);

struct BmeBuffers {
    DevBuf<double> T;
    DevBuf<int32_t> itab;
    DevBuf<double> out;
    DevBuf<int32_t> omove;
    int64_t cap_n = 0, ld = 0, ldi = 0;
    int64_t allocations = 0;
    int64_t launches = 0, evaluations = 0;
    double table_ms = 0, select_ms = 0;
    DevBuf<int32_t> spr_tab;
    DevBuf<double> spr_gain;
    DevBuf<int32_t> spr_wk;
    DevBuf<double> spr_dstack;
    DevBuf<int32_t> spr_istack;
    int64_t spr_ldi = 0;
    int64_t spr_allocations = 0;
    int64_t spr_launches = 0;
    double spr_scan_ms = 0;
};

struct UpgmaBuffers {
    DevBuf<double> D;
    DevBuf<double> size;
    DevBuf<uint64_t> nkey;
    DevBuf<int32_t> nn;
    DevBuf<int32_t> list;
    DevBuf<int32_t> log_x, log_y;
    DevBuf<double> log_h;
    DevBuf<char> st;
    int64_t cap_n = 0, ld = 0;
    int64_t allocations = 0;
    int64_t launches = 0, rescanned = 0;
    double loop_ms = 0;
};

struct MashIndex {
    uint32_t* post = nullptr;
    uint64_t* uniq = nullptr;
    uint32_t* off = nullptr;
    uint32_t* bkt = nullptr;
    uint32_t* ubase = nullptr;
    int32_t* shift = nullptr;
    uint64_t* vmax = nullptr;
    uint16_t* mult = nullptr;
    double* dtab = nullptr;
    int32_t* dblk = nullptr;
    uint16_t* dense = nullptr;
    int64_t chunks = 0;
    uint32_t nu = 0, ndense = 0;
};

struct MashBuffers {
    uint64_t* packed2 = nullptr;
    uint64_t* word_off = nullptr;
    uint64_t* len = nullptr;
    uint64_t* sketches = nullptr;
    uint4* tokens = nullptr;
    int32_t* tok_cnt = nullptr;
    uint64_t* ref = nullptr;
    int ref_n = 0;
    double tok_mean = 0.0;
    MashIndex index;
    bool share_chip = false;
    uint64_t total_words = 0;
    int64_t n = 0;
    int S = 0, k = 0;
};
int mash_upload(MashBuffers& m, const uint64_t* packed2, const uint64_t* word_off, const uint64_t* len,
                int64_t n, hipStream_t s);
void mash_free(MashBuffers& m);
int mash_sketch(MashBuffers& m, int k, int S, hipStream_t s);
int mash_dist_rows(const MashBuffers& m, int64_t r0, int64_t nr, int rank, int world, bool full,
                   int64_t ncols, double* out, int64_t ld, hipStream_t s, bool transposed = false);
int mash_dist_jobs(const MashBuffers& m, const PairJobs& J, int njobs, hipStream_t s);
int mash_index_build(MashBuffers& m, hipStream_t s);
void mash_index_free(MashIndex& ix);
void mash_index_info(const MashIndex& ix, int64_t info[8]);
int mash_dist_index(const MashBuffers& m, int64_t r0, int64_t nr, int64_t ncols, double* out, int64_t ld, double* mir,
                    bool transposed, hipStream_t s, int rank, int world);
int mash_dist_matrix_sharded(const MashBuffers& m, int rank, int world, int64_t rows_local, double* D_local, int64_t ld, hipStream_t s);
int mash_jobs_rows();
int mash_jobs_cols();
int mash_hash_positions(const MashBuffers& m, int64_t seq, int k, uint64_t* d_out, uint64_t len, uint64_t word_off,
                        hipStream_t s);

constexpr int64_t kNoDiag = (int64_t)1 << 40;
// ... 145 lines not shown
```

### dipper_amd/csrc/njp.hip

```cpp
#include "njp_args.hpp"

#include <algorithm>
#include <chrono>
#include <cstdio>
#include <cstdlib>
#include <functional>
#include <numeric>
#include <string>
#include <type_traits>

namespace dpr {

static int64_t njp_big_p()
{
    static const int64_t v = std::getenv("DPR_NJ_BIG_P") ? std::atoll(std::getenv("DPR_NJ_BIG_P")) : 40000;
    return v;
}
static bool njp_post2_on()
{
    static const bool on = !(std::getenv("DPR_NJP_POST2") && std::atoi(std::getenv("DPR_NJP_POST2")) == 0);
    return on;
}
static int njp_tg(int64_t P) { return P < njp_big_p() ? 64 : 256; }
constexpr int kBigNS = 4;
static int njp_ns(int64_t P) { return P < njp_big_p() ? 1 : kBigNS; }
__host__ __device__ inline int64_t njp_strips_of_rows(int64_t g0, int64_t tg, int64_t P)
{
    const int64_t G16 = (P + 16 - 1) / 16;
    const int64_t glast = (g0 + tg < G16 ? g0 + tg : G16) - 1;
    if (glast < 0) return 0;
    int64_t c = glast / 32 + 1;
    const int64_t cp = (P - 2) / 512 + 1;
    return P >= 2 ? (c < cp ? c : cp) : 0;
}

int njp_unit_owner(int64_t strip, int64_t group, int64_t P, int world)
{
    const int64_t G16 = (P + kUR - 1) / kUR;
    if (strip < 0 || group < 0 || group >= G16 || group < 32 * strip || strip * kTileCols >= P - 1 || world < 1) return -1;
    int64_t t = 0;
    const int64_t tg = njp_tg(P), ns = njp_ns(P);
    if (ns == 1) {
        for (int64_t c = 0; c < strip; ++c) t += (G16 - 32 * c + tg - 1) / tg;
        t += (group - 32 * strip) / tg;
    } else {
        const int64_t k = group / tg;
        for (int64_t kk = 0; kk < k; ++kk) t += (njp_strips_of_rows(kk * tg, tg, P) + ns - 1) / ns;
        t += strip / ns;
    }
    return (int)(t % world);
}

__device__ __forceinline__ void njp_note_range(unsigned long long* mm, double lo, double hi)
{
    if (lo < 0.0) {
        const double cur = dec_f64(mm[0]);
        if (cur >= 0.0 || lo < 2.0 * cur) atomicMin(&mm[0], (unsigned long long)enc_f64(lo));
    }
    if (hi > 0.0) {
        const double cur = dec_f64(mm[1]);
        if (hi > 2.0 * cur) atomicMax(&mm[1], (unsigned long long)enc_f64(hi));
    }
}

__global__ __launch_bounds__(kThreads) void njp_permute_kernel(const double* __restrict__ A, int64_t lda,
                                                               double* __restrict__ B, int64_t ldb,
                                                               const int32_t* __restrict__ perm, int64_t P)
{
    const int xcd = (int)(blockIdx.x & 7u), chunk = (int)(blockIdx.x >> 3), nchunk = (int)(gridDim.x >> 3);
    for (int64_t a = (int64_t)blockIdx.y * 8 + xcd; a < P; a += (int64_t)gridDim.y * 8) {
        const double* row = A + (int64_t)perm[a] * lda;
        for (int64_t b = (int64_t)chunk * kThreads + threadIdx.x; b < P; b += (int64_t)nchunk * kThreads)
            B[a * ldb + b] = row[perm[b]];
    }
}

static void njp_launch_permute(const double* A, int64_t lda, double* B, int64_t ldb, const int32_t* perm, int64_t n, hipStream_t s)
{
    int64_t chunks = (n + 1023) / 1024;
    chunks = chunks < 1 ? 1 : (chunks > 64 ? 64 : chunks);
    const int64_t gy = (n + 7) / 8;
    dim3 grid((unsigned)(8 * chunks), (unsigned)(gy < 32768 ? gy : 32768));
    hipLaunchKernelGGL(njp_permute_kernel, grid, dim3(kThreads), 0, s, A, lda, B, ldb, perm, n);
}

__global__ __launch_bounds__(kThreads) void njp_range_kernel(const double* __restrict__ A, int64_t lda, int64_t n, unsigned long long* __restrict__ mm)
{
    __shared__ double slo[kThreads / 64], shi[kThreads / 64];
    double lo = __builtin_inf(), hi = 0.0;
    for (int64_t a = blockIdx.x; a < n; a += gridDim.x) {
        const double* row = A + a * lda;
        for (int64_t b = threadIdx.x; b < n; b += kThreads) {
            const double v = row[b];
            lo = fmin(lo, v); hi = fmax(hi, fabs(v));
        }
    }
    lo = wave_fmin(lo); hi = wave_fmax(hi);
    if ((threadIdx.x & 63) == 0) { slo[threadIdx.x >> 6] = lo; shi[threadIdx.x >> 6] = hi; }
    __syncthreads();
    if (threadIdx.x == 0) {
        for (int w = 1; w < kThreads / 64; ++w) { lo = fmin(lo, slo[w]); hi = fmax(hi, shi[w]); }
        atomicMin(&mm[0], (unsigned long long)enc_f64(lo));
        atomicMax(&mm[1], (unsigned long long)enc_f64(hi));
    }
}

__global__ __launch_bounds__(kThreads) void njp_init_vectors_kernel(const double* __restrict__ U_src,
                                                                    const int32_t* __restrict__ perm,
                                                                    const int32_t* __restrict__ slot_src,
                                                                    int64_t P, int64_t n, double* __restrict__ U,
                                                                    double* __restrict__ Ur, uint64_t* __restrict__ KA,
                                                                    uint64_t* __restrict__ KB,
                                                                    int32_t* __restrict__ slot_of_pos,
                                                                    int32_t* __restrict__ pos_of_slot)
{
    const int64_t p = (int64_t)blockIdx.x * kThreads + threadIdx.x;
    if (p >= P) return;
    const int32_t src = perm[p];
    const int32_t slot = slot_src ? slot_src[src] : src;
    const double u = U_src[src];
    U[p] = u;
    Ur[p] = u / (double)(n - 2);
    KA[p] = nj_key_a_dev(slot, n);
    KB[p] = nj_key_b(slot);
    slot_of_pos[p] = slot;
    pos_of_slot[slot] = (int32_t)p;
}

__global__ void njp_fill_u64_kernel(uint64_t* __restrict__ a, int64_t cnt, uint64_t v)
{
    for (int64_t i = (int64_t)blockIdx.x * blockDim.x + threadIdx.x; i < cnt; i += (int64_t)gridDim.x * blockDim.x) a[i] = v;
}

__global__ __launch_bounds__(kThreads) void njp_list_all_kernel(NjpArgs a)
{
    const int tid = threadIdx.x;
    const int64_t it = a.st->it;
    if (a.st->status != 0) return;
    const int tb = a.sh_rank + (int)blockIdx.x * a.sh_world;
    const int cb0 = a.blk_cb[tb];
    const int64_t g = (int64_t)a.blk_g0[tb] + tid;
    const int64_t G16 = (a.P + kUR - 1) / kUR;
    const int tg = a.tg;
    int64_t send = njp_strips_of_rows((int64_t)a.blk_g0[tb], tg, a.P);
    if (a.ns == 1) send = cb0 + 1;
    else if (send > cb0 + a.ns) send = cb0 + a.ns;
    const int lane = tid & 63;
    for (int cb = cb0; cb < (int)send; ++cb) {
        const bool keep = g < G16 && g >= 32 * (int64_t)cb && tid < tg;
        const unsigned long long mask = __ballot(keep);
        unsigned long long base = 0;
        if (lane == 0 && mask) base = atomicAdd(&a.cnt[it % 3], (unsigned long long)__popcll(mask));
        base = __shfl(base, 0, 64);
        if (keep) a.list[base + __popcll(mask & ((1ull << lane) - 1ull))] = (int32_t)((0xFu << 28) | ((uint32_t)cb << 18) | (uint32_t)g);
    }
// ... 869 lines not shown
        }
        if (lead) {
            sUa = Uc[ci]; sUb = Uc[cj];
            const double xa = rowx[ci], ya = rowy[ci], xb = rowx[cj], yb = rowy[cj];
            const double ua = nj_unew(sUa, xa, ya, nj_val(xa, ya, d)) / r1;
            const double ub = nj_unew(sUb, xb, yb, nj_val(xb, yb, d)) / r1;
            const double qk = fmin((cand.d - ua) - ub, (cand.d - ub) - ua);
            qc = qk == qk ? qk : qc;
        }
    }
    ulonglong2 um0[kNS], um1[kNS];
    auto load_um = [&](int k) {
        const ulonglong2* up = reinterpret_cast<const ulonglong2*>(a.umin + ((int64_t)(cb0 + k) * G16 + g) * 8);
        const ulonglong2 p0 = up[0], p1 = up[1], p2 = up[2], p3 = up[3];
        um0[k] = make_ulonglong2(p0.x < p0.y ? p0.x : p0.y, p1.x < p1.y ? p1.x : p1.y);
        um1[k] = make_ulonglong2(p2.x < p2.y ? p2.x : p2.y, p3.x < p3.y ? p3.x : p3.y);
    };
#pragma unroll
    for (int k = 0; k < kNS; ++k) { um0[k] = make_ulonglong2(0ull, 0ull); um1[k] = um0[k]; }
    if (kNS == 1 && nsb > 0 && have_g && g >= 32 * (int64_t)cb0) load_um(0);
    qc = wave_fmin(qc);
    if (lane == 0) sseed[tid >> 6] = qc;
    NJP_STAMP(1, 3, true);
    const double slack = emin >= 0.0 ? 0.0 : (3.0 * -emin) * (1.0 + 0x1p-30) + eabs * 0x1p-47;
    const bool zlive = pz >= 0 && pz != px && pz != py;
    uz = (uz == uz) ? uz : PINF;
    const int64_t gz = zlive ? pz / kUR : -1;
    const int64_t sz = zlive ? pz / (kTileCols / 4) : -1;
    double rU = rmaxU;
    if (have_g && g == gz) rU = fmax(rU, uz);
    const double rmax = (rU + slack) / r1;
    if (tid < 4 * kNS) {
        double cU = cmU;
        if (4 * (int64_t)(cb0 + (tid >> 2)) + (tid & 3) == sz) cU = fmax(cU, uz);
        scm[tid] = (cU + slack) / r1;
    }
    const bool fold = zlive;
    const bool gz_here = fold && gz >= g0 && gz < g0 + kTG;
    const int wpz = fold ? (int)((pz % kTileCols) / (kTileCols / 4)) : -1;
    const int64_t cbz = fold ? pz / kTileCols : -1;
    const bool pz_here = fold && cbz >= cb0 && cbz < cb0 + nsb;
    double rC = wave_fmax(rmax);
    if (lane == 0) srC[tid >> 6] = rC;
    __syncthreads();
    const double bound = fmin(fmin(sseed[0], sseed[1]), fmin(sseed[2], sseed[3]));
    double cm4[kNS][4];
#pragma unroll
    for (int k = 0; k < kNS; ++k)
#pragma unroll
        for (int w = 0; w < 4; ++w) cm4[k][w] = scm[4 * k + w];
    {
        rC = fmax(fmax(srC[0], srC[1]), fmax(srC[2], srC[3]));
        double cC = NINF;
#pragma unroll
        for (int k = 0; k < kNS; ++k)
#pragma unroll
            for (int w = 0; w < 4; ++w) cC = fmax(cC, cm4[k][w]);
        const double lbC = fmin((cmin - rC) - cC, (cmin - cC) - rC);
        if (!gz_here && !pz_here && !(lbC <= bound)) {
            NJP_STAMP(1, 6, false);
            if (a.dbg != nullptr && it == a.dbg_it && tid == 0) a.dbg[(2048 + bx) * 8 + 7] = 3ull;
            return;
        }
        NJP_STAMP(1, 4, false);
    }
    double colz = PINF;
    if (gz_here && tid < 4 * kNS && (tid >> 2) < nsb) colz = a.t2_colmin[par * SS4 + 4 * (cb0 + (tid >> 2)) + (tid & 3)];
    if (kNS > 1) {
#pragma unroll
        for (int k = 0; k < kNS; ++k) {
            if (k < nsb && have_g && g >= 32 * (int64_t)(cb0 + k)) load_um(k);
        }
    }
    NJP_STAMP(1, 5, true);
    if (gz_here) {
        if (tid < 4 * kNS) s_colmin[tid] = colz;
        __syncthreads();
    }
    double mymin = PINF;
    int sub[kNS];
#pragma unroll
    for (int sidx = 0; sidx < kNS; ++sidx) {
        sub[sidx] = 0;
        if (sidx >= nsb) continue;
        const int cb = cb0 + sidx;
        const bool pz_strip = fold && cbz == cb;
        const bool have = have_g && g >= 32 * (int64_t)cb;
        ulonglong2* up4 = reinterpret_cast<ulonglong2*>(a.umin + ((int64_t)cb * G16 + (have ? g : 0)) * 8);
        double u4[4] = { PINF, PINF, PINF, PINF };
        if (have) { u4[0] = dec_f64(um0[sidx].x); u4[1] = dec_f64(um0[sidx].y); u4[2] = dec_f64(um1[sidx].x); u4[3] = dec_f64(um1[sidx].y); }
        const double newminA = (pz_strip && have_g) ? a.t2_rowmin[par * GS + g] : PINF;
        int submask = 0;
        if (have) {
#pragma unroll
            for (int w = 0; w < 4; ++w) {
                const double cmw = cm4[sidx][w];
                double nm = (gz_here && g == gz) ? s_colmin[4 * sidx + w] : PINF;
                if (pz_strip && w == wpz) nm = fmin(nm, newminA);
                if (nm < u4[w]) {
                    u4[w] = nm;
                    up4[w] = make_ulonglong2(enc_f64(nm), enc_f64(nm));
                }
                mymin = fmin(mymin, u4[w]);
                const double lb = fmin((u4[w] - rmax) - cmw, (u4[w] - cmw) - rmax);
                if ((cmw > NINF) && (lb <= bound)) submask |= 1 << w;
            }
        }
        if (have && (rmax > NINF)) sub[sidx] = submask;
    }
    NJP_STAMP(2, 0, false);
    {
        unsigned long long masks[kNS];
        int total = 0;
#pragma unroll
        for (int sidx = 0; sidx < kNS; ++sidx) { masks[sidx] = __ballot(sub[sidx] != 0); total += __popcll(masks[sidx]); }
        if (total > 0) {
            unsigned long long base = 0;
            if (lane == 0) base = atomicAdd(&a.cnt[(it + 1) % 3], (unsigned long long)total);
            base = __shfl(base, 0, 64);
            NJP_STAMP(2, 1, false);
#pragma unroll
            for (int sidx = 0; sidx < kNS; ++sidx) {
                if (sub[sidx] != 0)
                    a.list[base + __popcll(masks[sidx] & ((1ull << lane) - 1ull))] =
                        (int32_t)(((uint32_t)sub[sidx] << 28) | ((uint32_t)(cb0 + sidx) << 18) | (uint32_t)g);
                base += (unsigned long long)__popcll(masks[sidx]);
            }
        }
    }
    NJP_STAMP(2, 2, false);
    mymin = wave_fmin(mymin);
    __syncthreads();
    if (lane == 0) srC[tid >> 6] = mymin;
    __syncthreads();
    NJP_STAMP(2, 3, false);
    if (tid == 0) a.t2_cmin[tb] = fmin(fmin(srC[0], srC[1]), fmin(srC[2], srC[3]));
    NJP_STAMP(1, 6, true);
    if (a.dbg != nullptr && it == a.dbg_it && tid == 0) a.dbg[(2048 + bx) * 8 + 7] = 4ull;
}

static int64_t round_up16(int64_t v) { return (v + 15) / 16 * 16; }
static unsigned long long* g_njp_dbg_last = nullptr;

[[maybe_unused]] static const void* const kNjpInstantiations[] = {
    (const void*)njp_scan_kernel<false, 2>, (const void*)njp_post2_kernel<kBigNS>, (const void*)njp_post_kernel<64, 1, false>, (const void*)njp_post_kernel<256, kBigNS, false>,
    (const void*)njp_scan_kernel<true, 1>, (const void*)njp_post_kernel<64, 1, true>, (const void*)njp_finish_kernel<true>, (const void*)njp_finish_kernel<false> };

int njp_launch_list_all(const NjpArgs& a, hipStream_t s)
{
    if (a.ntest > 0) hipLaunchKernelGGL(njp_list_all_kernel, dim3((unsigned)a.ntest), dim3(kThreads), 0, s, a);
    DPR_HIP(hipGetLastError());
    return DPR_OK;
}
int njp_launch_scan(const NjpArgs& a, hipStream_t s)
{
    const int nrl = a.do_rows ? a.nrb : 0;
    auto* kernel = a.rs_world > 0 ? njp_scan_kernel<true, 1> : njp_scan_kernel<false, 2>;
    if (a.halves != (a.rs_world > 0 ? 1 : 2)) { set_error("njp_launch_scan: record layout does not match the kernel"); return DPR_ERR_STATE; }
    hipLaunchKernelGGL(kernel, dim3((unsigned)(a.halves * a.ugrid + nrl)), dim3(kThreads), 0, s, a.st, (const int32_t*)a.list, (const unsigned long long*)a.cnt,
                       (const double*)a.xpart, nrl, a);
    DPR_HIP(hipGetLastError());
    return DPR_OK;
}
int njp_launch_post(const NjpArgs& a0, int64_t N, bool post2, hipStream_t s)
{
    NjpArgs a = a0;
    unsigned ublocks = a.do_update ? (unsigned)((N + kThreads - 1) / kThreads) : 0u;
    if (post2 && a.do_update) {
        const unsigned u2 = (unsigned)((N + 2 * kThreads - 1) / (2 * kThreads));
        ublocks = u2 > (unsigned)a.nrb ? u2 : (unsigned)a.nrb;
    }
    a.nupd = (int)ublocks;
    if ((unsigned)a.ntest + ublocks == 0u) return DPR_OK;
    auto* kernel = a.rs_world > 0 ? njp_post_kernel<64, 1, true> : post2 ? njp_post2_kernel<kBigNS>
                 : a.tg == 64 ? njp_post_kernel<64, 1, false> : njp_post_kernel<256, kBigNS, false>;
    hipLaunchKernelGGL(kernel, dim3((unsigned)a.ntest + ublocks), dim3(kThreads), 0, s, a.st, (const NjRecord*)a.partials, (const unsigned long long*)a.cnt,
                       a.blk_cb, a.blk_g0, (const int32_t*)a.pos_of_slot, a.ntest, a.nupd, a);
    DPR_HIP(hipGetLastError());
    return DPR_OK;
}
int njp_launch_finish(const NjpArgs& a, hipStream_t s)
{
    auto* kernel = a.rs_world > 0 ? njp_finish_kernel<true> : njp_finish_kernel<false>;
    hipLaunchKernelGGL(kernel, dim3((unsigned)a.nrb), dim3(kThreads), 0, s, a);
    DPR_HIP(hipGetLastError());
    return DPR_OK;
}

static bool njp_use_post2(const NjPruned& q)
{
    const int ns = njp_ns(q.P);
    return njp_post2_on() && ns == kBigNS && (q.dbg == nullptr || q.dbg_it >= 0);
}

static size_t align256(size_t v) { return (v + 255) / 256 * 256; }
static int prep_blocks(int64_t P, int rs_world, int rs_rank, std::vector<int32_t>& hcb, std::vector<int32_t>& hg0)
{
    const int64_t G16 = (P + kUR - 1) / kUR;
    auto add = [&](int64_t c, int64_t g0) { hcb.push_back((int32_t)c); hg0.push_back((int32_t)g0); };
    if (rs_world > 1) {
        const int64_t gpc = kNjrChunk / kUR;
        for (int64_t c = 0; 32 * c < G16 && c * kTileCols < P - 1; ++c)
            for (int64_t g0 = (32 * c) / gpc * gpc; g0 < G16; g0 += gpc)
                if (njr_owner(g0 * kUR, rs_world) == rs_rank) add(c, g0);
    } else if (njp_ns(P) == 1) {
        for (int64_t c = 0; 32 * c < G16 && c * kTileCols < P - 1; ++c)
            for (int64_t g0 = 32 * c; g0 < G16; g0 += njp_tg(P)) add(c, g0);
    } else {
        for (int64_t g0 = 0; g0 < G16; g0 += njp_tg(P))
            for (int64_t c0 = 0; c0 < njp_strips_of_rows(g0, njp_tg(P), P); c0 += njp_ns(P)) add(c0, g0);
    }
    const int blocks = (int)hcb.size();
    if (blocks == 0) add(0, 0);
    return rs_world > 1 ? blocks : (int)hcb.size();
}
static int64_t vec_len(int64_t N) { return (N + kTileCols + 16 + 31) / 32 * 32; }

static int njp_carve(NjPruned* qp, char* slab, int64_t P, int64_t N, int local_ranks, hipStream_t s, size_t* total)
{
    NjPruned dry;
    NjPruned& q = slab ? *qp : dry;
    const size_t vec = (size_t)vec_len(N);
    const int64_t G16 = (P + kUR - 1) / kUR, S = (P + kTileCols - 1) / kTileCols + 1;
    size_t off = 0;
    hipError_t err = hipSuccess;
    auto take = [&](auto*& ptr, size_t count, int fill = -1) {
        using T = std::remove_reference_t<decltype(*ptr)>;
        if (slab) {
            ptr = reinterpret_cast<T*>(slab + off);
            if (fill >= 0 && err == hipSuccess) err = hipMemsetAsync(ptr, fill, count * sizeof(T), s);
        }
        off += align256(count * sizeof(T));
    };
    q.vstride = (int64_t)vec;
    take(q.U, 2 * vec, 0xff);
    take(q.R, 2 * vec, 0);
    take(q.Ur, vec, 0xff);
    take(q.KA, vec, 0);
    take(q.KB, vec, 0);
    take(q.slot_of_pos, vec, 0xff);
    take(q.pos_of_slot, vec, 0xff);
    take(q.perm, vec);
    q.nunits_alloc = S * G16 * 8;
    take(q.umin, (size_t)q.nunits_alloc);
    q.list_stride = unit_total(P) + kScanBlocks + 64;
    take(q.list, (size_t)(q.list_stride * local_ranks), 0);
    size_t nprep = 1;
    for (int64_t c = 0; 32 * c < G16 && c * kTileCols < P - 1; ++c) nprep += (size_t)((G16 - 32 * c + 31) / 32);
    take(q.blk_cb, nprep);
    take(q.blk_g0, nprep);
    take(q.cnt_all, (size_t)(4 * local_ranks), 0);
    take(q.t2_hdr, 256);
    take(q.t2_rmax, (size_t)(2 * 32 * (S + 1)));
    take(q.t2_rowmin, (size_t)(2 * 32 * (S + 1)));
    take(q.t2_cmax, (size_t)(2 * 4 * (S + 1)));
    take(q.t2_colmin, (size_t)(2 * 4 * (S + 1)));
    take(q.t2_cmin, nprep);
    *total = off;
    return err == hipSuccess ? DPR_OK : hip_fail(err, "hipMemsetAsync (epoch slab)");
}
static size_t matrix_bytes(int64_t N)
{
    const int64_t rows_alloc = (N + kRowBlock - 1) / kRowBlock * kRowBlock + 32;
    return (size_t)(rows_alloc * round_up16(N) + kTileCols + 16) * sizeof(double);
}

static int njp_local_ranks(const NjPruned& q) { return q.sh_world > 1 && q.sh_virtual ? q.sh_world : 1; }

static int njp_reserve_slabs(NjPruned& q, int64_t N, int local_ranks, bool with_matrix, hipStream_t s)
{
    size_t total = 0;
    if (int rc = njp_carve(nullptr, nullptr, N, N, local_ranks, nullptr, &total)) return rc;
    if (q.arena_slab[0] && (q.arena_D || !with_matrix) && q.arena_N == N && q.arena_ranks >= local_ranks && q.arena_slab_bytes >= total) return DPR_OK;
    void* old[] = { with_matrix ? q.arena_D : nullptr, q.arena_slab[0], q.arena_slab[1] };
    for (void* p : old)
        if (p) (void)hipFree(p);
    q.arena_slab[0] = q.arena_slab[1] = nullptr;
    if (with_matrix) {
        q.arena_D = nullptr;
        DPR_HIP(hipMalloc(&q.arena_D, matrix_bytes(N)));
        DPR_HIP(hipMemsetAsync(q.arena_D, 0, matrix_bytes(N), s));
    }
    for (int k = 0; k < 2; ++k) DPR_HIP(hipMalloc(&q.arena_slab[k], total));
    q.arena_slab_bytes = total; q.arena_N = N; q.arena_ranks = local_ranks;
    return DPR_OK;
}

int njp_arena(NjPruned& q, int64_t N, hipStream_t s) { return njp_reserve_slabs(q, N, njp_local_ranks(q), true, s); }

static int njp_alloc_epoch(NjPruned& q, int64_t P, int64_t N, double* Dbuf, char* slab, hipStream_t s, const void* hdr_from = nullptr,
                           int rs_world = 1, int rs_rank = 0)
{
    if (P >= (int64_t)kTileCols * 1024) { set_error("pruned NJ: the list encoding holds fewer than 524288 positions"); return DPR_ERR_ARG; }
    q.P = P;
    q.ld = round_up16(P);
    q.D = Dbuf;
    const int64_t rows_alloc = (P + kUR - 1) / kUR * kUR + kUR;
    if (rs_world <= 1)
        if (int rc = nj_fill_pads(q.D, q.ld, P, P, rows_alloc, kTileCols + 16, false, s)) return rc;
    std::vector<int32_t> hcb, hg0;
    q.nprep = prep_blocks(P, rs_world, rs_rank, hcb, hg0);
    q.utot = unit_total(P);
    size_t total = 0;
    if (int rc = njp_carve(&q, slab, P, N, njp_local_ranks(q), s, &total)) return rc;
    if (hdr_from != nullptr) {
        DPR_HIP(hipMemcpyAsync(q.t2_hdr, hdr_from, 16, hipMemcpyDeviceToDevice, s));
    } else {
        const unsigned long long h0[2] = { 0xFFF0000000000000ull , 0x8000000000000000ull  };
        DPR_HIP(hipMemcpyAsync(q.t2_hdr, h0, sizeof h0, hipMemcpyHostToDevice, s));
        DPR_HIP(hipStreamSynchronize(s));
    }
    DPR_HIP(hipMemcpyAsync(q.blk_cb, hcb.data(), sizeof(int32_t) * hcb.size(), hipMemcpyHostToDevice, s));
    DPR_HIP(hipMemcpyAsync(q.blk_g0, hg0.data(), sizeof(int32_t) * hg0.size(), hipMemcpyHostToDevice, s));
    DPR_HIP(hipStreamSynchronize(s));
    hipLaunchKernelGGL(njp_fill_u64_kernel, dim3(256), dim3(256), 0, s, (uint64_t*)q.umin, q.nunits_alloc,
                       enc_f64_host(-__builtin_inf()));
    hipLaunchKernelGGL(njp_fill_u64_kernel, dim3(16), dim3(256), 0, s, (uint64_t*)q.t2_cmin, (int64_t)q.nprep, 0xFFF0000000000000ull);
    DPR_HIP(hipGetLastError());
    q.fresh = true;
    return DPR_OK;
}

int njp_rs_epoch(NjPruned& q, int64_t P, int64_t N, double* Dbuf, int epoch_index, int rs_rank, int rs_world, const void* hdr_from, hipStream_t s)
{
    if (int rc = njp_reserve_slabs(q, N, 1, false, s)) return rc;
    if (q.graph) { (void)hipGraphExecDestroy(q.graph); q.graph = nullptr; }
    q.sh_world = 1; q.sh_rank = 0; q.sh_virtual = false;
    q.epoch_index = epoch_index;
    if (int rc = njp_alloc_epoch(q, P, N, Dbuf, q.arena_slab[epoch_index & 1], s, hdr_from, rs_world, rs_rank)) return rc;
    q.active = true;
    return DPR_OK;
}

int njp_epoch_order(const double* dU, const int32_t* slot_of_pos, int64_t P, int64_t n, std::vector<int32_t>& perm, bool stream_idle, hipStream_t s)
{
    std::vector<double> hU((size_t)P);
    if (stream_idle) {
        DPR_HIP(hipMemcpy(hU.data(), dU, sizeof(double) * (size_t)P, hipMemcpyDeviceToHost));
    } else {
        DPR_HIP(hipMemcpyAsync(hU.data(), dU, sizeof(double) * (size_t)P, hipMemcpyDeviceToHost, s));
        DPR_HIP(hipStreamSynchronize(s));
    }
    perm.clear();
    perm.reserve((size_t)n);
    if (slot_of_pos) {
        std::vector<int32_t> hslot((size_t)P);
        DPR_HIP(hipMemcpy(hslot.data(), slot_of_pos, sizeof(int32_t) * (size_t)P, hipMemcpyDeviceToHost));
        for (int64_t p = 0; p < P; ++p)
            if (hslot[(size_t)p] >= 0) perm.push_back((int32_t)p);
    } else {
        perm.resize((size_t)P);
        std::iota(perm.begin(), perm.end(), 0);
    }
    if ((int64_t)perm.size() != n) { set_error("pruned NJ epoch: live positions do not match the active size"); return DPR_ERR_STATE; }
    std::stable_sort(perm.begin(), perm.end(), [&](int32_t a, int32_t c) {
        const double ua = hU[(size_t)a], uc = hU[(size_t)c];
        if (ua != ua) return false;
        if (uc != uc) return true;
        return ua < uc;
    });
    return DPR_OK;
}
int njp_init_vectors(NjPruned& q, const double* U_src, const int32_t* slot_src, int64_t n, int64_t it, hipStream_t s)
{
    hipLaunchKernelGGL(njp_init_vectors_kernel, dim3((unsigned)((n + kThreads - 1) / kThreads)), dim3(kThreads), 0, s,
                       U_src, (const int32_t*)q.perm, slot_src, n, n, q.U + (it & 1) * q.vstride, q.Ur, q.KA, q.KB, q.slot_of_pos, q.pos_of_slot);
    DPR_HIP(hipGetLastError());
    return DPR_OK;
}
int njp_put_fresh_state(NjState* d_st, NjState& st, hipStream_t s)
{
    st.pnew[0] = -1; st.pnew[1] = -1;
    for (auto& c : st.cnt_list) c = 0ull;
    DPR_HIP(hipMemcpyAsync(d_st, &st, sizeof(NjState), hipMemcpyHostToDevice, s));
    return DPR_OK;
}
static int njp_find_range(NjPruned& q, const double* D, int64_t ld, int64_t n, hipStream_t s)
{
    q.range_known = njp_use_post2(q);
    if (!q.range_known) return DPR_OK;
    hipLaunchKernelGGL(njp_range_kernel, dim3(2048), dim3(kThreads), 0, s, D, ld, n, (unsigned long long*)q.t2_hdr);
    DPR_HIP(hipGetLastError());
    return DPR_OK;
}
void njp_plan_from_env(NjPruned& q)
{
    const char* e = std::getenv("DPR_NJP_GRID");
    const int g = e ? std::atoi(e) : 512;
    q.scan_grid = g < 1 ? 1 : (g > 1024 ? 1024 : g);
    if (const char* gi = std::getenv("DPR_NJ_GRAPH_ITERS")) { const int v = std::atoi(gi); if (v >= 1 && v <= 4096) q.graph_iters = v; }
}

int njp_build(NjBuffers& b, hipStream_t s)
{
    NjPruned& q = b.pr;
    njp_plan_from_env(q);
    if (const char* e = std::getenv("DPR_NJ_ADAPTIVE")) q.adaptive = std::atoi(e) != 0 ? 1 : 0;
    if (const char* e = std::getenv("DPR_NJ_STREAM_FRAC")) q.stream_frac = std::atof(e);
    q.stream_iterations = 0; q.stream_epochs = 0;
    if (const char* e = std::getenv("DPR_NJ_PHASES")) {
        q.dbg_it = std::atoll(e);
        if (!q.dbg) DPR_HIP(hipMalloc(&q.dbg, sizeof(unsigned long long) * 4 * 2048 * 8));
        DPR_HIP(hipMemsetAsync(q.dbg, 0, sizeof(unsigned long long) * 4 * 2048 * 8, s));
        g_njp_dbg_last = q.dbg;
    }
    const int64_t N = b.N;
    std::vector<int32_t> perm;
    if (int rc = njp_epoch_order(b.U, nullptr, N, N, perm, false, s)) return rc;
    if (int rc = njp_arena(q, N, s)) return rc;
    q.epoch_index = 0;
    if (int rc = njp_alloc_epoch(q, N, N, q.arena_D, q.arena_slab[0], s)) return rc;
    q.utot0 = q.utot;
    DPR_HIP(hipMemcpyAsync(q.perm, perm.data(), sizeof(int32_t) * (size_t)N, hipMemcpyHostToDevice, s));
    njp_launch_permute(b.D, b.ld, q.D, q.ld, q.perm, N, s);
    if (int rc = njp_find_range(q, b.D, b.ld, N, s)) return rc;
    if (int rc = njp_init_vectors(q, b.U, nullptr, N, 0, s)) return rc;
    DPR_HIP(hipStreamSynchronize(s));
    q.active = true;
    return DPR_OK;
}

static int njp_rebuild_epoch(NjBuffers& b, hipStream_t s, bool* rebuilt)
{
    NjPruned& q = b.pr;
    *rebuilt = false;
    const bool tlog = log_level("epoch") >= 3;
    auto tprev = std::chrono::steady_clock::now();
    auto lap = [&](const char* what) {
        if (!tlog) return;
        const auto t = std::chrono::steady_clock::now();
        std::fprintf(stderr, "[njp]   rebuild: %s %.3f ms\n", what, std::chrono::duration<double, std::milli>(t - tprev).count());
        tprev = t;
    };
    NjState st;
    DPR_HIP(hipMemcpy(&st, b.st, sizeof(NjState), hipMemcpyDeviceToHost));
    const int64_t n = st.n;
    if (st.status != 0 || n < 3) return DPR_OK;
    const double* Ucur = njp_current_u(q, st.it);
    std::vector<int32_t> perm;
    if (int rc = njp_epoch_order(Ucur, q.slot_of_pos, q.P, n, perm, true, s)) return rc;
    lap("state + vectors to the host, sort");
    if (q.graph) { (void)hipGraphExecDestroy(q.graph); q.graph = nullptr; }
    const NjPruned old = q;
    const int e = old.epoch_index + 1;
    q.epoch_index = e;
    if (int rc = njp_alloc_epoch(q, n, b.N, (e & 1) ? b.D : q.arena_D, q.arena_slab[e & 1], s, old.range_known ? old.t2_hdr : nullptr)) return rc;
    lap("njp_alloc_epoch");
    DPR_HIP(hipMemcpyAsync(q.perm, perm.data(), sizeof(int32_t) * (size_t)n, hipMemcpyHostToDevice, s));
    njp_launch_permute(old.D, old.ld, q.D, q.ld, q.perm, n, s);
    if (int rc = njp_init_vectors(q, Ucur, old.slot_of_pos, n, st.it, s)) return rc;
    if (int rc = njp_put_fresh_state(b.st, st, s)) return rc;
    lap("enqueue");
    DPR_HIP(hipStreamSynchronize(s));
    lap("device work");
    *rebuilt = true;
    return DPR_OK;
}

__global__ __launch_bounds__(kThreads) void njp_gather_u_kernel(const double* __restrict__ Ucur, const int32_t* __restrict__ pos_of_slot,
                                                                int64_t n, double* __restrict__ U)
{
    const int64_t s = (int64_t)blockIdx.x * kThreads + threadIdx.x;
    if (s < n) U[s] = Ucur[pos_of_slot[s]];
}

static int njp_to_slots(NjBuffers& b, hipStream_t s)
{
    NjPruned& q = b.pr;
    NjState st;
    DPR_HIP(hipMemcpy(&st, b.st, sizeof(NjState), hipMemcpyDeviceToHost));
    const int64_t n = st.n;
    if (st.status != 0 || n < 3) return DPR_OK;
    if (q.graph) { (void)hipGraphExecDestroy(q.graph); q.graph = nullptr; }
    if (q.D == b.D) std::swap(b.D, q.arena_D);
    njp_launch_permute((const double*)q.D, q.ld, b.D, b.ld, (const int32_t*)q.pos_of_slot, n, s);
    hipLaunchKernelGGL(njp_gather_u_kernel, dim3((unsigned)((n + kThreads - 1) / kThreads)), dim3(kThreads), 0, s,
                       njp_current_u(q, st.it), (const int32_t*)q.pos_of_slot, n, b.U);
    DPR_HIP(hipGetLastError());
    if (int rc = nj_prepare(b, s)) return rc;
    q.slots_mode = true;
    ++q.stream_epochs;
    return DPR_OK;
}

static int njp_from_slots(NjBuffers& b, hipStream_t s)
{
    NjPruned& q = b.pr;
    NjState st;
    DPR_HIP(hipStreamSynchronize(s));
    DPR_HIP(hipMemcpy(&st, b.st, sizeof(NjState), hipMemcpyDeviceToHost));
    const int64_t n = st.n;
    if (st.status != 0 || n < 3) return DPR_OK;
    std::vector<int32_t> perm;
    if (int rc = njp_epoch_order(b.U, nullptr, n, n, perm, true, s)) return rc;
    q.epoch_index = 0;
    if (int rc = njp_alloc_epoch(q, n, b.N, q.arena_D, q.arena_slab[0], s)) return rc;
    DPR_HIP(hipMemcpyAsync(q.perm, perm.data(), sizeof(int32_t) * (size_t)n, hipMemcpyHostToDevice, s));
    njp_launch_permute((const double*)b.D, b.ld, q.D, q.ld, (const int32_t*)q.perm, n, s);
    if (int rc = njp_find_range(q, b.D, b.ld, n, s)) return rc;
    if (int rc = njp_init_vectors(q, b.U, nullptr, n, st.it, s)) return rc;
    if (int rc = njp_put_fresh_state(b.st, st, s)) return rc;
    DPR_HIP(hipStreamSynchronize(s));
    q.slots_mode = false;
    return DPR_OK;
}

static int njp_run_slots(NjBuffers& b, int64_t it0, int64_t todo, hipStream_t s)
{
    const int64_t n0 = b.N - it0;
    for (int64_t k = 0; k < todo; ++k) {
        if (int rc = nj_launch_scan(b, false, n0 - k, it0 + k, s)) return rc;
        if (int rc = nj_launch_post(b, n0 - k, it0 + k, s)) return rc;
    }
    b.pr.stream_iterations += todo;
    return nj_launch_finish(b, n0 - todo, it0 + todo, s);
}

void njp_reset(NjPruned& q)
{
    if (q.graph) { (void)hipGraphExecDestroy(q.graph); q.graph = nullptr; }
    NjPruned fresh;
    fresh.arena_D = q.arena_D; fresh.arena_slab[0] = q.arena_slab[0]; fresh.arena_slab[1] = q.arena_slab[1];
    fresh.arena_slab_bytes = q.arena_slab_bytes; fresh.arena_N = q.arena_N; fresh.arena_ranks = q.arena_ranks;
    fresh.adaptive = q.adaptive;
    fresh.dbg = q.dbg;
    q = fresh;
}

void njp_free(NjPruned& q)
{
    njp_reset(q);
    if (q.dbg) { if (g_njp_dbg_last == q.dbg) g_njp_dbg_last = nullptr; (void)hipFree(q.dbg); q.dbg = nullptr; }
    void* ptrs[] = { q.arena_D, q.arena_slab[0], q.arena_slab[1] };
    for (void* p : ptrs)
        if (p) (void)hipFree(p);
    q = NjPruned();
}

constexpr int kNjpHalves = 2;
static int njp_grid_rank(const NjPruned& q) { return q.sh_world > 1 ? (q.scan_grid / q.sh_world > 0 ? q.scan_grid / q.sh_world : 1) : q.scan_grid; }
static int njp_grid_total(const NjPruned& q) { return q.sh_world > 1 ? njp_grid_rank(q) * q.sh_world : q.scan_grid; }
static int njp_first_rank(const NjPruned& q) { return q.sh_world > 1 && !q.sh_virtual ? q.sh_rank : 0; }
static int njp_last_rank(const NjPruned& q) { return q.sh_world > 1 ? (q.sh_virtual ? q.sh_world : q.sh_rank + 1) : 1; }

static NjpArgs njp_args(NjBuffers& b, int v)
{
    NjPruned& q = b.pr;
    const bool sh = q.sh_world > 1;
    const int slot = sh && q.sh_virtual ? v : 0;
    NjpArgs a{};
    a.D = q.D; a.ld = q.ld; a.st = b.st;
    a.U = q.U; a.R = q.R; a.vstride = q.vstride;
    a.Ur = q.Ur; a.KA = q.KA; a.KB = q.KB; a.slot_of_pos = q.slot_of_pos; a.pos_of_slot = q.pos_of_slot;
    a.xpart = b.xpart; a.partials = b.partials; a.umin = (unsigned long long*)q.umin;
    a.P = q.P;
    a.blk_cb = q.blk_cb; a.blk_g0 = q.blk_g0;
    a.tg = njp_tg(q.P); a.ns = njp_ns(q.P); a.nupd = 0;
    a.ntest = sh ? (q.nprep - v + q.sh_world - 1) / q.sh_world : q.nprep;
    a.list = q.list + (int64_t)slot * q.list_stride;
    a.cnt = sh ? q.cnt_all + 4 * slot : b.st->cnt_list;
    a.ugrid = njp_grid_rank(q);
    a.halves = kNjpHalves;
    a.urecs = kNjpHalves * njp_grid_total(q);
    a.nrb = (int)((q.P + kTileCols - 1) / kTileCols);
    a.rec_off = sh ? v * kNjpHalves * a.ugrid : 0;
    a.all_defined = sh ? 1 : 0;
    a.sh_rank = sh ? v : 0; a.sh_world = sh ? q.sh_world : 1;
    a.cnt_all = sh ? q.cnt_all : nullptr;
    a.cnt_ranks = sh ? (q.sh_virtual ? q.sh_world : 1) : 0;
    a.do_update = 1; a.do_tests = 1; a.do_rows = 1;
    a.log_x = b.log_x; a.log_y = b.log_y; a.log_bx = b.log_bx; a.log_by = b.log_by;
    a.dbg = q.dbg; a.dbg_it = q.dbg_it;
    a.t2_hdr = q.t2_hdr; a.t2_rmax = q.t2_rmax; a.t2_cmax = q.t2_cmax; a.t2_colmin = q.t2_colmin; a.t2_rowmin = q.t2_rowmin; a.t2_cmin = q.t2_cmin;
    return a;
}

static int njp_enqueue_iteration(NjBuffers& b, hipStream_t s, bool sample = false)
{
    NjPruned& q = b.pr;
    const bool post2 = njp_use_post2(q);
    if (q.sh_world <= 1) {
        const NjpArgs a = njp_args(b, 0);
        if (sample) { b.kt->nk = 3; njp_set_kernel_names(nullptr); }
        if (int rc = nj_timing_mark(b.kt, sample, s)) return rc;
        if (int rc = njp_launch_scan(a, s)) return rc;
        if (int rc = nj_timing_mark(b.kt, sample, s)) return rc;
        if (int rc = njp_launch_post(a, b.N, post2, s)) return rc;
        if (int rc = nj_timing_mark(b.kt, sample, s)) return rc;
        return nj_timing_mark(b.kt, sample, s);
    }
    const int v0 = njp_first_rank(q), v1 = njp_last_rank(q);
    for (int v = v0; v < v1; ++v) {
        NjpArgs a = njp_args(b, v);
        a.do_rows = v == v0 ? 1 : 0;
        if (int rc = njp_launch_scan(a, s)) return rc;
    }
    if (!q.sh_virtual) {
        if (!q.gather) { set_error("njp: unit-sharded mode without a gather callback"); return DPR_ERR_STATE; }
        if (int rc = q.gather(q.gather_ctx, b.partials, sizeof(NjRecord) * (size_t)(kNjpHalves * njp_grid_rank(q)), s)) return rc;
    }
    for (int v = v0; v < v1; ++v) {
        NjpArgs a = njp_args(b, v);
        a.do_update = v == v0 ? 1 : 0;
        if (int rc = njp_launch_post(a, b.N, post2, s)) return rc;
    }
    return DPR_OK;
}

int njp_capture_graph(NjPruned& q, hipStream_t s, const std::function<int()>& enqueue)
{
    const auto t0 = std::chrono::steady_clock::now();
    ScopedGraph g;
    DPR_HIP(hipStreamBeginCapture(s, hipStreamCaptureModeThreadLocal));
    int rc = DPR_OK;
    for (int k = 0; k < q.graph_iters && rc == DPR_OK; ++k) rc = enqueue();
    hipError_t e = hipStreamEndCapture(s, g.put());
    if (rc != DPR_OK) return rc;
    if (e != hipSuccess) return hip_fail(e, "hipStreamEndCapture");
    e = hipGraphInstantiate(&q.graph, g, nullptr, nullptr, 0);
    if (e != hipSuccess) { q.graph = nullptr; return hip_fail(e, "hipGraphInstantiate"); }
    if (log_level("epoch") > 0)
        std::fprintf(stderr, "[njp] graph capture + instantiate (P=%lld): %.2f ms\n", (long long)q.P,
                     std::chrono::duration<double, std::milli>(std::chrono::steady_clock::now() - t0).count());
    return DPR_OK;
}

static int njp_run_segment(NjBuffers& b, int64_t it0, int64_t todo, hipStream_t s)
{
    NjPruned& q = b.pr;
    const int64_t limit = it0 + todo;
    DPR_HIP(hipMemcpyAsync(&b.st->it_limit, &limit, sizeof(int64_t), hipMemcpyHostToDevice, s));
    DPR_HIP(hipStreamSynchronize(s));
    if (todo <= 0) return DPR_OK;
    const int v0 = njp_first_rank(q), v1 = njp_last_rank(q);
    if (q.fresh) {
        for (int v = v0; v < v1; ++v)
            if (int rc = njp_launch_list_all(njp_args(b, v), s)) return rc;
        if (njp_use_post2(q)) {
            const int64_t S2 = (q.P + kTileCols - 1) / kTileCols + 2;
            const int par = (int)(it0 & 1);
            hipLaunchKernelGGL(njp_t2_init_kernel, dim3((unsigned)((q.P + kTileCols - 1) / kTileCols)), dim3(kThreads), 0, s,
                               (const double*)njp_current_u(q, it0), q.P, q.t2_rmax + par * 32 * S2, q.t2_cmax + par * 4 * S2);
            DPR_HIP(hipGetLastError());
        }
        q.fresh = false;
    }
    const bool timing = b.kt && b.kt->stride > 0 && q.sh_world <= 1;
    const bool use_graph = q.sh_world <= 1 && todo >= q.graph_iters && !timing;
    if (use_graph && !q.graph)
        if (int rc = njp_capture_graph(q, s, [&] { return njp_enqueue_iteration(b, s); })) return rc;
    int64_t done = 0;
    if (use_graph)
        for (; done + q.graph_iters <= todo; done += q.graph_iters) DPR_HIP(hipGraphLaunch(q.graph, s));
    for (; done < todo; ++done)
        if (int rc = njp_enqueue_iteration(b, s, timing && (it0 + done) % b.kt->stride == 0)) return rc;
    return njp_launch_finish(njp_args(b, v0), s);
}

static const char* const kNjpKernelNames[] = { "njp_scan_kernel", "njp_post_kernel", "(empty event pair)", "" };
static const char* const* g_kernel_names = kNjpKernelNames;
void njp_set_kernel_names(const char* const* names) { g_kernel_names = names ? names : kNjpKernelNames; }
const char* njp_kernel_name(int idx)
{
    if (idx < 0 || idx >= kNjKernelsMax) return "";
    for (int k = 0; k <= idx; ++k)
        if (g_kernel_names[k][0] == 0) return "";
    return g_kernel_names[idx];
}

int njp_debug_list(NjBuffers& b, int32_t* out, int64_t cap, int64_t* count, int64_t* P, double* ur, int64_t urcap)
{
    NjPruned& q = b.pr;
    if (!q.active || q.slots_mode || q.sh_world > 1) { set_error("njp_debug_list: no single-rank pruned epoch"); return DPR_ERR_STATE; }
    DPR_HIP(hipDeviceSynchronize());
    NjState st;
    DPR_HIP(hipMemcpy(&st, b.st, sizeof(NjState), hipMemcpyDeviceToHost));
    const int64_t cnt = (int64_t)st.cnt_list[st.it % 3];
    *count = cnt; *P = q.P;
    const int64_t take = cnt < cap ? cnt : cap;
    if (take > 0) DPR_HIP(hipMemcpy(out, q.list, sizeof(int32_t) * (size_t)take, hipMemcpyDeviceToHost));
    const int64_t tu = q.P < urcap ? q.P : urcap;
    if (ur && tu > 0) DPR_HIP(hipMemcpy(ur, q.Ur, sizeof(double) * (size_t)tu, hipMemcpyDeviceToHost));
    return DPR_OK;
}

int njp_phase_stamps(unsigned long long* out)
{
    if (!g_njp_dbg_last) { set_error("DPR_NJ_PHASES not set"); return DPR_ERR_STATE; }
    DPR_HIP(hipDeviceSynchronize());
    DPR_HIP(hipMemcpy(out, g_njp_dbg_last, sizeof(unsigned long long) * 4 * 2048 * 8, hipMemcpyDeviceToHost));
    return DPR_OK;
}

const double* njp_current_u(const NjPruned& q, int64_t it) { return q.U + (it & 1) * q.vstride; }

int njp_shape(const NjPruned& q, int64_t* positions, int* row_groups, int* strips, int* post2, int* scan_grid)
{
    if (positions) *positions = q.P;
    if (row_groups) *row_groups = njp_tg(q.P);
    if (strips) *strips = njp_ns(q.P);
    if (post2) *post2 = njp_use_post2(q) ? 1 : 0;
    if (scan_grid) *scan_grid = q.scan_grid;
    return DPR_OK;
}

constexpr int64_t kEpochPct = 80;
int64_t njp_epoch_min()
{
    const char* e = std::getenv("DPR_NJ_EPOCH_MIN");
    return e ? std::atoll(e) : 2048;
}
bool njp_epoch_due(int64_t P, int64_t n, int64_t left, int64_t epoch_min, int64_t* seg)
{
    *seg = left;
    if (epoch_min <= 0 || P < epoch_min) return false;
    const int64_t target = P * kEpochPct / 100;
    if (n <= target && n >= 3) return true;
    if (n - target < left) *seg = n - target;
    return false;
}

int njp_run(NjBuffers& b, int64_t it0, int64_t todo, hipStream_t s)
{
    const int64_t epoch_min = njp_epoch_min();
    NjPruned& q = b.pr;
    int64_t it = it0, left = todo;
    if (left <= 0) return q.slots_mode ? DPR_OK : njp_run_segment(b, it0, 0, s);
    while (left > 0) {
        const int64_t n = b.N - it;
        if (q.slots_mode) {
            if (n <= q.slots_probe_n && n >= epoch_min && n >= 3) {
                if (int rc = njp_from_slots(b, s)) return rc;
                if (!q.slots_mode) continue;
            }
            int64_t seg = left;
            if (n > q.slots_probe_n && q.slots_probe_n >= epoch_min && n - q.slots_probe_n < seg) seg = n - q.slots_probe_n;
            if (int rc = njp_run_slots(b, it, seg, s)) return rc;
            it += seg; left -= seg;
            continue;
        }
        int64_t seg = left;
        if (njp_epoch_due(q.P, n, left, epoch_min, &seg)) {
            DPR_HIP(hipStreamSynchronize(s));
            const auto t0 = std::chrono::steady_clock::now();
            bool rebuilt = false;
            if (int rc = njp_rebuild_epoch(b, s, &rebuilt)) return rc;
            if (!rebuilt) return DPR_OK;
            if (log_level("epoch") > 0)
                std::fprintf(stderr, "[njp] epoch rebuild at n=%lld: %.2f ms\n", (long long)n,
                             std::chrono::duration<double, std::milli>(std::chrono::steady_clock::now() - t0).count());
            continue;
        }
        const bool watch = q.adaptive && q.sh_world <= 1 && q.utot > 0;
        unsigned long long units0 = 0;
        bool first_of_epoch = false;
        if (watch) {
            first_of_epoch = q.fresh;
            const int64_t chunk = first_of_epoch ? (int64_t)q.graph_iters : 2048;
            if (seg > chunk) seg = chunk;
            NjState st0;
            DPR_HIP(hipStreamSynchronize(s));
            DPR_HIP(hipMemcpy(&st0, b.st, sizeof(NjState), hipMemcpyDeviceToHost));
            units0 = st0.units_scanned;
        }
        if (int rc = njp_run_segment(b, it, seg, s)) return rc;
        it += seg; left -= seg;
        if (watch && left > 0) {
            NjState st1;
            DPR_HIP(hipStreamSynchronize(s));
            DPR_HIP(hipMemcpy(&st1, b.st, sizeof(NjState), hipMemcpyDeviceToHost));
            if (st1.status != 0) continue;
            const double listed = (double)(st1.units_scanned - units0) - (first_of_epoch ? (double)q.utot : 0.0);
            const double iters = (double)seg - (first_of_epoch ? 1.0 : 0.0);
            const double rate = iters >= 1.0 ? listed / (iters * (double)q.utot) : 0.0;
            const double per_it = iters >= 1.0 ? listed / iters : 0.0;
            if (log_level("epoch") >= 2)
                std::fprintf(stderr, "[njp] watch at n=%lld: %.0f units per iteration over %.0f iterations (first of epoch %d, P=%lld, utot=%lld, scan grid %d)\n",
                             (long long)(b.N - it), per_it, iters, (int)first_of_epoch, (long long)q.P, (long long)q.utot, q.scan_grid);
            if (iters >= 1.0 && rate > q.stream_frac) {
                const int64_t na = b.N - it;
                int64_t pn = na;
                const int hops = 1 << (q.probe_fail_streak < 4 ? q.probe_fail_streak : 4);
                for (int h = 0; h < hops; ++h) pn = pn * kEpochPct / 100;
                ++q.probe_fail_streak;
                q.slots_probe_n = pn;
                if (int rc = njp_to_slots(b, s)) return rc;
                if (log_level("epoch") > 0)
                    std::fprintf(stderr, "[njp] %.0f %% of the units listed per iteration at n=%lld: handed over to the streaming loop; next pruned probe at n <= %lld\n",
                                 100.0 * rate, (long long)na, (long long)pn);
            } else if (!first_of_epoch) {
                q.probe_fail_streak = 0;
            }
        }
    }
    return DPR_OK;
}

}
```

### include/dipper_hip.h

```cpp
#ifndef DIPPER_HIP_H
#define DIPPER_HIP_H

#include <stdint.h>

#ifdef __cplusplus
extern "C" {
#endif
#pragma GCC visibility push(default)

#define DPR_ABI_VERSION 1
#define DPR_ROW_BLOCK 64

#define DPR_SRC_MSA 1
#define DPR_SRC_MASH 2
#define DPR_SRC_MATRIX 3

#define DPR_DIST_UNCORRECTED 1
#define DPR_DIST_JC 2
#define DPR_DIST_TAJIMANEI 3
#define DPR_DIST_K2P 4
#define DPR_DIST_TAMURA 5
#define DPR_DIST_JINNEI 6
#define DPR_DIST_POISSON 7
#define DPR_DIST_KIMURA 8
#define DPR_DIST_TN93 9
#define DPR_DIST_LOGDET 10
#define DPR_DIST_PARALINEAR 11

#define DPR_OK 0
#define DPR_ERR_ARG -1
#define DPR_ERR_HIP -2
#define DPR_ERR_STATE -3
#define DPR_ERR_NOCAND -4
#define DPR_ERR_COMM -5

typedef struct dpr_ctx dpr_ctx;

const char *dpr_last_error(void);
int dpr_abi_version(void);

int dpr_pack4(const char *seq, uint64_t len, uint64_t *out);
int dpr_pack2(const char *seq, uint64_t len, uint64_t *out);
int dpr_pack_aa(const char *seq, uint64_t len, uint8_t *out);

#define DPR_NJR_CHUNK 1024
int dpr_njr_owner(int64_t position, int world);
int64_t dpr_njr_local_row(int64_t position, int world);
int64_t dpr_njr_global_pos(int64_t local_row, int rank, int world);
int64_t dpr_njr_rows_cap(int64_t positions, int world);
int dpr_shard_owner(int64_t row, int world);
int64_t dpr_shard_local_row(int64_t row, int world);
int64_t dpr_shard_rows(int64_t n, int rank, int world);
int64_t dpr_shard_global_row(int64_t local, int rank, int world);
int dpr_record_reduce(const void *records, int count);
uint64_t dpr_nj_key(int64_t i, int64_t j, int64_t n);

int dpr_create(dpr_ctx **out, int device);
int dpr_destroy(dpr_ctx *ctx);
int dpr_create_virtual(dpr_ctx **out, int device, int world);
int dpr_device_name(dpr_ctx *ctx, char *buf, int cap);

int dpr_comm_unique_id(void *out128);
int dpr_comm_init(dpr_ctx *ctx, int rank, int world, const void *id128);
int dpr_comm_selftest(dpr_ctx *ctx);
int dpr_comm_init_local(dpr_ctx *ctx, int rank, int world);
int dpr_peer_export(dpr_ctx *ctx, int64_t n_tips, void *out192);
int dpr_peer_attach(dpr_ctx *ctx, const void *all192);
int dpr_comm_info(dpr_ctx *ctx, int *rank, int *nranks);
#define DPR_COMM_SHARED_BYTES 65536
int dpr_comm_init_shared(dpr_ctx *ctx, int rank, int world, void *shared, uint64_t bytes, int transport);
int dpr_comm_stats(dpr_ctx *ctx, int *transport, int64_t *collectives);
int dpr_shared_abort(void *shared);
int dpr_shared_failed(const void *shared);
int dpr_shared_barrier(void *shared, int world, uint32_t *sense, int timeout_ms);
int dpr_shared_gather(void *shared, int rank, int world, uint32_t *sense, int timeout_ms, const void *mine, void *all, int bytes);

int dpr_set_msa(dpr_ctx *ctx, const uint64_t *packed4, int64_t n, int64_t L);
int dpr_set_msa_aa(dpr_ctx *ctx, const uint8_t *codes, int64_t n, int64_t L);
int dpr_set_reads(dpr_ctx *ctx, const uint64_t *packed2, const uint64_t *word_off,
                  const uint64_t *len, int64_t n);
int dpr_set_matrix_lower(dpr_ctx *ctx, const double *rows, int64_t n);

int dpr_sketch(dpr_ctx *ctx, int k, int S, uint64_t *host_sketches);
int dpr_get_mash_index_info(dpr_ctx *ctx, int64_t info[8]);

int dpr_dist_matrix(dpr_ctx *ctx, int source, int dist_type, int k);

int dpr_warm_graphs(dpr_ctx *ctx);

int dpr_reserve_nj(dpr_ctx *ctx, int64_t n);

int64_t dpr_nj_run(dpr_ctx *ctx, int64_t max_iters, int32_t *merge_x, int32_t *merge_y,
                   double *bl_x, double *bl_y, double *last_d);

int dpr_argmin_once(dpr_ctx *ctx, int reps, int32_t *out_i, int32_t *out_j, double *out_q,
                    float *out_ms_per_scan);

int dpr_set_nj_mode(int mode);
int dpr_set_nj_virtual_shards(int w);
int dpr_set_nj_multi_plan(int plan);
int dpr_nj_is_unit_sharded(dpr_ctx *ctx);
int dpr_get_nj_multi_info(dpr_ctx *ctx, char *buf, int cap);
#define DPR_NJ_PLAN_SINGLE_STREAM 0
#define DPR_NJ_PLAN_SINGLE_PRUNED 1
#define DPR_NJ_PLAN_BIONJ 2
#define DPR_NJ_PLAN_ROWS_STREAM 3
#define DPR_NJ_PLAN_REPLICAS 4
#define DPR_NJ_PLAN_UNIT_SHARDED 5
#define DPR_NJ_PLAN_ROWS_PRUNED 6
int dpr_nj_plan_resolve(int world, int virtual_ranks, int variant, int pruned, int multi_plan, int virtual_shards, int64_t n,
                        uint64_t total_bytes);
int dpr_ctx_set_nj_mode(dpr_ctx *ctx, int mode);
int dpr_ctx_set_nj_multi_plan(dpr_ctx *ctx, int plan);
int dpr_ctx_set_nj_adaptive(dpr_ctx *ctx, int on);
int dpr_get_nj_adaptive_stats(dpr_ctx *ctx, int64_t *stream_iterations, int64_t *stream_epochs);
int dpr_ctx_set_nj_exchange(dpr_ctx *ctx, int plan);
int dpr_ctx_set_debug_fault(dpr_ctx *ctx, int64_t iteration, int rank);
int dpr_get_nj_exchange_info(dpr_ctx *ctx, int *active_plan, int64_t *launches, int64_t *collectives, char *note, int cap);
int dpr_ctx_set_poll_limit_ms(dpr_ctx *ctx, int ms);
int dpr_ctx_set_nj_virtual_shards(dpr_ctx *ctx, int w);
int dpr_ctx_set_nj_variant(dpr_ctx *ctx, int variant);
int dpr_get_nj_lambda(dpr_ctx *ctx, double *out , int64_t *count);
int64_t dpr_nj_variant_host(int variant, const double *lower_rows, int64_t n, int64_t max_iters,
                            int32_t *merge_x, int32_t *merge_y, double *bl_x, double *bl_y,
                            double *last_d, double *lambda );
int dpr_ctx_set_nj_kernel_timing(dpr_ctx *ctx, int stride);
int dpr_get_nj_kernel_timing(dpr_ctx *ctx, int *kernels, double *us_avg4, int64_t *samples);
const char *dpr_nj_kernel_name(int idx);
int dpr_get_nj_phase_stamps(uint64_t *out32768);
int dpr_get_njp_list(dpr_ctx *ctx, int32_t *out, int64_t cap, int64_t *count, int64_t *positions, double *ur, int64_t ur_cap);
int dpr_njp_unit_owner(int64_t strip, int64_t group, int64_t P, int world);
int dpr_get_prune_stats(dpr_ctx *ctx, uint64_t *units_scanned, uint64_t *units_per_full_scan);
int dpr_get_nj_progress(dpr_ctx *ctx, int64_t *iterations_done, int64_t *active);
int dpr_get_njp_shape(dpr_ctx *ctx, int64_t *positions, int *row_groups, int *strips, int *post2, int *scan_grid);

int dpr_launch_bench(dpr_ctx *ctx, int nlaunch, int grid, int use_graph, float *us_per_launch);
int dpr_spin_start(dpr_ctx *ctx, int blocks, int max_ms);
int dpr_spin_stop(dpr_ctx *ctx);

int dpr_scan_tune(int rows_per_unit, int nontemporal, int grid);

int dpr_bw_probe(dpr_ctx *ctx, int64_t bytes, int nontemporal, int grid, int reps, float *out_ms);

int64_t dpr_n_active(dpr_ctx *ctx);
int64_t dpr_n_total(dpr_ctx *ctx);
int dpr_get_matrix_row(dpr_ctx *ctx, int64_t i, double *out );
int dpr_get_row_sums(dpr_ctx *ctx, double *out );
int dpr_get_msa_counts(dpr_ctx *ctx, int64_t row, int32_t *useful, int32_t *match );
int dpr_msa_dist_block(dpr_ctx *ctx, int64_t row0, int64_t nrows, int64_t ncols, int dist_type, int transposed, double *out,
                       int reps, float *ms_avg);
int dpr_get_kmer_hashes(dpr_ctx *ctx, int64_t seq, int k, const uint64_t *word_off, const uint64_t *len,
                        uint64_t *out);
int dpr_get_place_state(dpr_ctx *ctx, int32_t *cid, double *cdis, double *trace);
int dpr_get_timing(dpr_ctx *ctx, double *dist_ms, double *nj_ms);

int dpr_place_run(dpr_ctx *ctx, int source, int dist_type, int k, int64_t first, int64_t n,
                  int32_t *head, int32_t *e, int32_t *nxt, int32_t *belong, double *len);

int dpr_get_place_timing(dpr_ctx *ctx, double *dist_ms, double *tree_ms);
int dpr_get_place_overlap(dpr_ctx *ctx, int *overlapped, double *dist_busy_ms);
int dpr_get_place_policy(dpr_ctx *ctx, int64_t *batches, int64_t *overlapped_batches);
int dpr_place_policy_run(int source, int world, int window_transport, int no_overlap, int64_t multi_min, int64_t first, int64_t last,
                         int64_t batch_rows, const double *tree_ms, const double *dist_alone_ms, int64_t batches, int32_t *beside);

int dpr_get_place_walks(dpr_ctx *ctx, int32_t *reached , int64_t *stats6);

int dpr_place_exact_run(dpr_ctx *ctx, int source, int dist_type, int k, int64_t n, int32_t *head, int32_t *e,
                        int32_t *nxt, int32_t *belong, double *len);
int dpr_get_exact_state(dpr_ctx *ctx, int32_t *rev, int32_t *dep);

#define DPR_DC_EXACT_LAST 1
#define DPR_DC_VIRTUAL_RANKS(w) (((w) & 0xff) << 8)
int dpr_dc_run(dpr_ctx *ctx, int source, int dist_type, int k, int64_t n, int64_t backbone, int flags,
               int32_t *head, int32_t *e, int32_t *nxt, int32_t *belong, double *len, int32_t *cluster_id);
int dpr_dc_query_share(int64_t n, int64_t backbone, int rank, int world, int64_t *q0, int64_t *q1);
int dpr_dc_deal_clusters(const int64_t *sizes_desc, int64_t count, int world, int32_t *owner);
int dpr_get_dc_stats(dpr_ctx *ctx, int64_t *counts5, double *phase_ms3);
int dpr_get_dc_table_stats(dpr_ctx *ctx, int64_t out4[4]);

int dpr_place_fixed_set(dpr_ctx *ctx, int64_t m, int64_t n, const int32_t *head, const int32_t *e, const int32_t *nxt,
                        const int32_t *belong, const double *len);
int dpr_place_fixed_run(dpr_ctx *ctx, int source, int dist_type, int k, int32_t *slot, double *frac, double *add);
int dpr_ctx_set_place_fixed_batch(dpr_ctx *ctx, int64_t queries);
int dpr_get_place_fixed_timing(dpr_ctx *ctx, double *dist_ms, double *scan_ms);

int dpr_get_msa_site_coverage(dpr_ctx *ctx, int32_t *out);
int64_t dpr_msa_filter_sites(dpr_ctx *ctx, int permille);

int dpr_msa_resample(dpr_ctx *ctx, uint64_t seed, int64_t replicate);
int dpr_get_msa_boot_weights(dpr_ctx *ctx, int32_t *out);
int dpr_msa_boot_weights(uint64_t seed, int64_t replicate, int64_t L, int32_t *out);
int dpr_split_support(int64_t n, const int32_t *main_x, const int32_t *main_y, const int32_t *rep_x, const int32_t *rep_y,
                      int32_t *counts);
int dpr_comm_sum_i32(dpr_ctx *ctx, int32_t *host_inout, int64_t count);

int dpr_transfer_support(dpr_ctx *ctx, int64_t n, const int32_t *main_x, const int32_t *main_y, const int32_t *rep_x,
                         const int32_t *rep_y, int64_t *phi_sum);
int dpr_transfer_support_host(int64_t n, const int32_t *main_x, const int32_t *main_y, const int32_t *rep_x, const int32_t *rep_y,
                              int64_t *phi_sum);
int dpr_transfer_taxa(dpr_ctx *ctx, int64_t n, const int32_t *main_x, const int32_t *main_y, const int32_t *rep_x,
                      const int32_t *rep_y, int cutoff_permille, int64_t *phi_sum, int64_t *moved, int64_t *pairs);
int dpr_transfer_taxa_host(int64_t n, const int32_t *main_x, const int32_t *main_y, const int32_t *rep_x, const int32_t *rep_y,
                           int cutoff_permille, int64_t *phi_sum, int64_t *moved, int64_t *pairs);
int dpr_ctx_set_tbe_lds(dpr_ctx *ctx, int64_t bytes);
int dpr_comm_sum_i64(dpr_ctx *ctx, int64_t *host_inout, int64_t count);

int dpr_bme_nni(dpr_ctx *ctx, int64_t n, const int32_t *merge_x, const int32_t *merge_y, int max_rounds, int32_t *kids, int32_t *top,
                double *len, double *L_rounds, int64_t *stats4);
int dpr_bme_nni_host(const double *lower_rows, int64_t n, const int32_t *merge_x, const int32_t *merge_y, int max_rounds, int32_t *kids,
                     int32_t *top, double *len, double *L_rounds, int64_t *stats4);
int dpr_bme_eval_host(const double *lower_rows, int64_t n, const int32_t *kids, int32_t top, double *len, double *gain, int32_t *move,
                      double *L);
int dpr_get_bme_timing(dpr_ctx *ctx, double *table_ms, double *select_ms);
int dpr_get_bme_stats(dpr_ctx *ctx, int64_t *out4);

int dpr_bme_spr(dpr_ctx *ctx, int64_t n, const int32_t *merge_x, const int32_t *merge_y, int max_rounds, int32_t *kids, int32_t *top,
                double *len, double *L_rounds, int64_t *stats6);
int dpr_bme_spr_host(const double *lower_rows, int64_t n, const int32_t *merge_x, const int32_t *merge_y, int max_rounds, int32_t *kids,
                     int32_t *top, double *len, double *L_rounds, int64_t *stats6);
int dpr_bme_spr_eval_host(const double *lower_rows, int64_t n, const int32_t *kids, int32_t top, double *best_gain, int32_t *best_w,
                          int32_t *best_k, double *L);
int dpr_bme_spr_gain_host(const double *lower_rows, int64_t n, const int32_t *kids, int32_t top, int64_t d, int32_t w, double *gain,
                          int32_t *k);
int dpr_get_bme_spr_timing(dpr_ctx *ctx, double *scan_ms);
int dpr_get_bme_spr_stats(dpr_ctx *ctx, int64_t *out4);

int64_t dpr_upgma_run(dpr_ctx *ctx, int linkage, int32_t *merge_x, int32_t *merge_y, double *height);
int dpr_upgma_host(const double *lower_rows, int64_t n, int linkage, int32_t *merge_x, int32_t *merge_y, double *height);
int dpr_get_upgma_stats(dpr_ctx *ctx, int64_t *out4);
int dpr_get_upgma_timing(dpr_ctx *ctx, double *loop_ms);

#pragma GCC visibility pop
#ifdef __cplusplus
}
#endif
#endif
```

Before: 34140.

## Launch eager iterations ahead of the first graph capture in pruned NJ

Each pruned NJ segment now enqueues a lead of eager scan/post launches before capturing and instantiating the hipGraph. The lead is large for the first graph in the process and small afterward, so the one-time graph instantiation cost is hidden behind GPU work already in flight. The scan and post launch parameters are precomputed once per segment, so each eager iteration only fires two kernels. Warm-up graph capture is skipped for the pruned, BIONJ and replica plans, and blocking hipMemcpy calls are replaced with stream-ordered async copies followed by a sync. It also adds stats and segment-plan query APIs, at the cost of more eager launches on short runs.

```diff
diff --git a/dipper_amd/capi.py b/dipper_amd/capi.py
--- a/dipper_amd/capi.py
+++ b/dipper_amd/capi.py
@@ -79,6 +79,8 @@
     L.dpr_ctx_set_poll_limit_ms.argtypes = [C.c_void_p, C.c_int]
     L.dpr_ctx_set_nj_adaptive.argtypes = [C.c_void_p, C.c_int]
     L.dpr_get_nj_adaptive_stats.argtypes = [C.c_void_p, C.POINTER(C.c_int64), C.POINTER(C.c_int64)]
+    L.dpr_get_nj_graph_stats.argtypes = [C.c_void_p] + [C.POINTER(C.c_int64)] * 4
+    L.dpr_njp_segment_plan.argtypes = [C.c_int64, C.c_int64, C.c_int64] + [C.POINTER(C.c_int64)] * 3
     L.dpr_scan_tune.argtypes = [C.c_int, C.c_int, C.c_int]
     L.dpr_set_nj_mode.argtypes = [C.c_int]
     L.dpr_set_nj_multi_plan.argtypes = [C.c_int]
@@ -251,6 +253,13 @@
  NJ_PLAN_ROWS_PRUNED) = range(7)
 
 
+def njp_segment_plan(seg, lead, graph_len):
+    L = load_library()
+    v = [C.c_int64() for _ in range(3)]
+    _chk(L, L.dpr_njp_segment_plan(seg, lead, graph_len, *[C.byref(x) for x in v]))
+    return tuple(int(x.value) for x in v)
+
+
 def nj_plan_resolve(world, virtual_ranks, variant, pruned, multi_plan, virtual_shards, n, total_bytes):
     L = load_library()
     return _chk(L, L.dpr_nj_plan_resolve(world, int(virtual_ranks), variant, int(pruned), multi_plan, virtual_shards, n, total_bytes))
@@ -550,6 +559,11 @@
         b = C.c_int64()
         _chk(self.L, self.L.dpr_get_nj_adaptive_stats(self.h, C.byref(a), C.byref(b)))
         return int(a.value), int(b.value)
+
+    def nj_graph_stats(self):
+        v = [C.c_int64() for _ in range(4)]
+        _chk(self.L, self.L.dpr_get_nj_graph_stats(self.h, *[C.byref(x) for x in v]))
+        return {"graphs": int(v[0].value), "replayed": int(v[1].value), "eager": int(v[2].value), "lead_seen": int(v[3].value)}
 
     def set_debug_fault(self, iteration, rank):
         _chk(self.L, self.L.dpr_ctx_set_debug_fault(self.h, iteration, rank))
diff --git a/dipper_amd/csrc/ctx_nj.hip b/dipper_amd/csrc/ctx_nj.hip
--- a/dipper_amd/csrc/ctx_nj.hip
+++ b/dipper_amd/csrc/ctx_nj.hip
@@ -277,12 +277,16 @@
         if (tlog) std::fprintf(stderr, "  dpr_warm_graphs: %s at %.1f ms\n", what, std::chrono::duration<double, std::milli>(std::chrono::steady_clock::now() - t0).count());
     };
     hipStream_t st = c->stream;
-    if (hipStreamBeginCapture(st, hipStreamCaptureModeThreadLocal) == hipSuccess) {
+    const int64_t n_known = c->nj.empty() ? 0 : c->nj[0].N;
+    const int kind = ctx_nj_plan(c, n_known >= 3 ? n_known : 3, "dpr_warm_graphs");
+    const bool behind_lead = kind == DPR_NJ_PLAN_SINGLE_PRUNED || kind == DPR_NJ_PLAN_BIONJ || (kind == DPR_NJ_PLAN_REPLICAS && n_known >= 3);
+    if (!behind_lead && hipStreamBeginCapture(st, hipStreamCaptureModeThreadLocal) == hipSuccess) {
         hipLaunchKernelGGL(dpr_warm_kernel, dim3(1), dim3(64), 0, st, 0);
         ScopedGraph g;
         ScopedGraphExec ge;
         if (hipStreamEndCapture(st, g.put()) == hipSuccess && g) {
             if (hipGraphInstantiate(ge.put(), g, nullptr, nullptr, 0) == hipSuccess && ge) {
+                njp_note_graph_instantiated();
                 lap("first hipGraphInstantiate");
                 (void)hipGraphLaunch(ge, st);
                 (void)hipStreamSynchronize(st);
@@ -319,6 +323,11 @@
 }
 extern "C" {
 
+static hipError_t stream_copy(void* dst, const void* src, size_t bytes, hipMemcpyKind k, hipStream_t s)
+{
+    const hipError_t e = hipMemcpyAsync(dst, src, bytes, k, s);
+    return e != hipSuccess ? e : hipStreamSynchronize(s);
+}
 int64_t dpr_nj_run(dpr_ctx* c, int64_t max_iters, int32_t* merge_x, int32_t* merge_y, double* bl_x,
                    double* bl_y, double* last_d)
 {
@@ -333,6 +342,7 @@
     c->nj[0].kt = &c->nj_kt;
     if (c->nj_kt.stride > 0 && it0 == 0) { c->nj_kt.samples = 0; for (double& v : c->nj_kt.us_sum) v = 0; }
     c->nj_launches = 0; c->nj_collectives = 0;
+    { NjPruned& q = c->nj[0].pr; q.run_graphs = 0; q.run_replayed = 0; q.run_eager = 0; q.run_lead_seen = -1; }
     DPR_HIP(hipEventRecord(c->ev[2], c->stream));
     if (c->plan.kind == DPR_NJ_PLAN_ROWS_PRUNED) {
         std::vector<NjBuffers*> ranks = njr_ranks(c);
@@ -376,10 +386,10 @@
     }
     const int64_t done = st.it - it0;
     if (done > 0) {
-        if (merge_x) DPR_HIP(hipMemcpy(merge_x, c->nj[0].log_x + it0, sizeof(int32_t) * (size_t)done, hipMemcpyDeviceToHost));
-        if (merge_y) DPR_HIP(hipMemcpy(merge_y, c->nj[0].log_y + it0, sizeof(int32_t) * (size_t)done, hipMemcpyDeviceToHost));
-        if (bl_x) DPR_HIP(hipMemcpy(bl_x, c->nj[0].log_bx + it0, sizeof(double) * (size_t)done, hipMemcpyDeviceToHost));
-        if (bl_y) DPR_HIP(hipMemcpy(bl_y, c->nj[0].log_by + it0, sizeof(double) * (size_t)done, hipMemcpyDeviceToHost));
+        if (merge_x) DPR_HIP(stream_copy(merge_x, c->nj[0].log_x + it0, sizeof(int32_t) * (size_t)done, hipMemcpyDeviceToHost, c->stream));
+        if (merge_y) DPR_HIP(stream_copy(merge_y, c->nj[0].log_y + it0, sizeof(int32_t) * (size_t)done, hipMemcpyDeviceToHost, c->stream));
+        if (bl_x) DPR_HIP(stream_copy(bl_x, c->nj[0].log_bx + it0, sizeof(double) * (size_t)done, hipMemcpyDeviceToHost, c->stream));
+        if (bl_y) DPR_HIP(stream_copy(bl_y, c->nj[0].log_by + it0, sizeof(double) * (size_t)done, hipMemcpyDeviceToHost, c->stream));
     }
     if (st.status == 3) {
         set_error("dpr_nj_run: the exchange between the ranks failed (a rank's record did not arrive within the poll limit, or the all-gather delivered a stale one)");
@@ -404,18 +414,18 @@
     if (last_d && st.n == 2) {
         NjBuffers& b0 = c->nj[0];
         int32_t pos01[2] = { 0, 1 };
-        if (b0.pr.in_positions()) DPR_HIP(hipMemcpy(pos01, b0.pr.pos_of_slot, sizeof(pos01), hipMemcpyDeviceToHost));
+        if (b0.pr.in_positions()) DPR_HIP(stream_copy(pos01, b0.pr.pos_of_slot, sizeof(pos01), hipMemcpyDeviceToHost, c->stream));
         const double* row1 = slot_row(c, 1, pos01[1], true);
         const bool by_record = c->plan.rows_dealt() && c->vworld == 0 && c->plan.exchange == kNjsLegacy;
         if (row1 && !by_record) {
-            DPR_HIP(hipMemcpy(last_d, row1 + pos01[0], sizeof(double), hipMemcpyDeviceToHost));
+            DPR_HIP(stream_copy(last_d, row1 + pos01[0], sizeof(double), hipMemcpyDeviceToHost, c->stream));
         } else {
             NjRecord rec{ 0.0, 0ull, 0.0, 0ull };
-            if (row1) DPR_HIP(hipMemcpy(&rec.d, row1 + pos01[0], sizeof(double), hipMemcpyDeviceToHost));
-            DPR_HIP(hipMemcpy(b0.recs + c->rank, &rec, sizeof(NjRecord), hipMemcpyHostToDevice));
+            if (row1) DPR_HIP(stream_copy(&rec.d, row1 + pos01[0], sizeof(double), hipMemcpyDeviceToHost, c->stream));
+            DPR_HIP(stream_copy(b0.recs + c->rank, &rec, sizeof(NjRecord), hipMemcpyHostToDevice, c->stream));
             if (int rc = exchange(c, EX_RECS)) return rc;
             DPR_HIP(hipStreamSynchronize(c->stream));
-            DPR_HIP(hipMemcpy(&rec, b0.recs + 0, sizeof(NjRecord), hipMemcpyDeviceToHost));
+            DPR_HIP(stream_copy(&rec, b0.recs + 0, sizeof(NjRecord), hipMemcpyDeviceToHost, c->stream));
             *last_d = rec.d;
         }
     }
@@ -583,6 +593,23 @@
     if (!c || !c->have_matrix || !c->nj[0].pr.active) { set_error("dpr_get_nj_adaptive_stats: pruned path not active"); return DPR_ERR_STATE; }
     if (stream_iterations) *stream_iterations = c->nj[0].pr.stream_iterations;
     if (stream_epochs) *stream_epochs = c->nj[0].pr.stream_epochs;
+    return DPR_OK;
+}
+int dpr_get_nj_graph_stats(dpr_ctx* c, int64_t* graphs, int64_t* replayed, int64_t* eager, int64_t* lead_seen)
+{
+    if (!c || !c->have_matrix || !c->nj[0].pr.active) { set_error("dpr_get_nj_graph_stats: pruned path not active"); return DPR_ERR_STATE; }
+    const NjPruned& q = c->nj[0].pr;
+    if (graphs) *graphs = q.run_graphs;
+    if (replayed) *replayed = q.run_replayed;
+    if (eager) *eager = q.run_eager;
+    if (lead_seen) *lead_seen = q.run_lead_seen;
+    return DPR_OK;
+}
+int dpr_njp_segment_plan(int64_t seg, int64_t lead, int64_t graph_len, int64_t* head, int64_t* graphs, int64_t* tail)
+{
+    if (!head || !graphs || !tail) { set_error("dpr_njp_segment_plan: null argument"); return DPR_ERR_ARG; }
+    const NjpSegmentPlan p = njp_segment_plan(seg, lead, graph_len);
+    *head = p.head; *graphs = p.graphs; *tail = p.tail;
     return DPR_OK;
 }
 
diff --git a/dipper_amd/csrc/dpr_internal.hpp b/dipper_amd/csrc/dpr_internal.hpp
--- a/dipper_amd/csrc/dpr_internal.hpp
+++ b/dipper_amd/csrc/dpr_internal.hpp
@@ -94,6 +94,8 @@
     int32_t pnew[2];
 };
 
+constexpr int kNjpLeadFirst = 2016;
+constexpr int kNjpLeadNext = 64;
 struct NjPruned {
     bool active = false;
     int64_t P = 0, ld = 0;
@@ -125,6 +127,9 @@
     hipGraphExec_t graph = nullptr;
     int scan_grid = 512;
     int graph_iters = 32;
+    int lead_first = kNjpLeadFirst;
+    int lead_next = kNjpLeadNext;
+    int64_t run_graphs = 0, run_replayed = 0, run_eager = 0, run_lead_seen = -1;
     int adaptive = 1;
     double stream_frac = 0.7;
     bool slots_mode = false;
@@ -305,6 +310,9 @@
 void njp_reset(NjPruned& q);
 int njp_unit_owner(int64_t strip, int64_t group, int64_t P, int world);
 int njp_run(NjBuffers& b, int64_t it0, int64_t todo, hipStream_t s);
+struct NjpSegmentPlan { int64_t head = 0, graphs = 0, tail = 0; };
+NjpSegmentPlan njp_segment_plan(int64_t seg, int64_t lead, int64_t graph_len);
+void njp_note_graph_instantiated();
 const char* njp_kernel_name(int idx);
 void njp_set_kernel_names(const char* const* names);
 int njp_phase_stamps(unsigned long long* out);
diff --git a/dipper_amd/csrc/njp.hip b/dipper_amd/csrc/njp.hip
--- a/dipper_amd/csrc/njp.hip
+++ b/dipper_amd/csrc/njp.hip
@@ -1,6 +1,7 @@
 #include "njp_args.hpp"
 
 #include <algorithm>
+#include <atomic>
 #include <chrono>
 #include <cstdio>
 #include <cstdlib>
@@ -1176,30 +1177,64 @@
     DPR_HIP(hipGetLastError());
     return DPR_OK;
 }
-int njp_launch_scan(const NjpArgs& a, hipStream_t s)
-{
-    const int nrl = a.do_rows ? a.nrb : 0;
-    auto* kernel = a.rs_world > 0 ? njp_scan_kernel<true, 1> : njp_scan_kernel<false, 2>;
+struct NjpScanLaunch {
+    decltype(&njp_scan_kernel<false, 2>) kernel = nullptr;
+    unsigned grid = 0;
+    int nrl = 0;
+    NjpArgs a{};
+};
+struct NjpPostLaunch {
+    decltype(&njp_post_kernel<64, 1, false>) kernel = nullptr;
+    unsigned grid = 0;
+    NjpArgs a{};
+};
+static int njp_prepare_scan(const NjpArgs& a, NjpScanLaunch* l)
+{
     if (a.halves != (a.rs_world > 0 ? 1 : 2)) { set_error("njp_launch_scan: record layout does not match the kernel"); return DPR_ERR_STATE; }
-    hipLaunchKernelGGL(kernel, dim3((unsigned)(a.halves * a.ugrid + nrl)), dim3(kThreads), 0, s, a.st, (const int32_t*)a.list, (const unsigned long long*)a.cnt,
-                       (const double*)a.xpart, nrl, a);
-    DPR_HIP(hipGetLastError());
-    return DPR_OK;
-}
-int njp_launch_post(const NjpArgs& a0, int64_t N, bool post2, hipStream_t s)
-{
-    NjpArgs a = a0;
+    l->nrl = a.do_rows ? a.nrb : 0;
+    l->kernel = a.rs_world > 0 ? njp_scan_kernel<true, 1> : njp_scan_kernel<false, 2>;
+    l->grid = (unsigned)(a.halves * a.ugrid + l->nrl);
+    l->a = a;
+    return DPR_OK;
+}
+static inline void njp_fire(const NjpScanLaunch& l, hipStream_t s)
+{
+    hipLaunchKernelGGL(l.kernel, dim3(l.grid), dim3(kThreads), 0, s, l.a.st, (const int32_t*)l.a.list, (const unsigned long long*)l.a.cnt,
+                       (const double*)l.a.xpart, l.nrl, l.a);
+}
+static void njp_prepare_post(const NjpArgs& a0, int64_t N, bool post2, NjpPostLaunch* l)
+{
+    NjpArgs& a = l->a;
+    a = a0;
     unsigned ublocks = a.do_update ? (unsigned)((N + kThreads - 1) / kThreads) : 0u;
     if (post2 && a.do_update) {
         const unsigned u2 = (unsigned)((N + 2 * kThreads - 1) / (2 * kThreads));
         ublocks = u2 > (unsigned)a.nrb ? u2 : (unsigned)a.nrb;
     }
     a.nupd = (int)ublocks;
-    if ((unsigned)a.ntest + ublocks == 0u) return DPR_OK;
-    auto* kernel = a.rs_world > 0 ? njp_post_kernel<64, 1, true> : post2 ? njp_post2_kernel<kBigNS>
-                 : a.tg == 64 ? njp_post_kernel<64, 1, false> : njp_post_kernel<256, kBigNS, false>;
-    hipLaunchKernelGGL(kernel, dim3((unsigned)a.ntest + ublocks), dim3(kThreads), 0, s, a.st, (const NjRecord*)a.partials, (const unsigned long long*)a.cnt,
-                       a.blk_cb, a.blk_g0, (const int32_t*)a.pos_of_slot, a.ntest, a.nupd, a);
+    l->grid = (unsigned)a.ntest + ublocks;
+    l->kernel = a.rs_world > 0 ? njp_post_kernel<64, 1, true> : post2 ? njp_post2_kernel<kBigNS>
+              : a.tg == 64 ? njp_post_kernel<64, 1, false> : njp_post_kernel<256, kBigNS, false>;
+}
+static inline void njp_fire(const NjpPostLaunch& l, hipStream_t s)
+{
+    hipLaunchKernelGGL(l.kernel, dim3(l.grid), dim3(kThreads), 0, s, l.a.st, (const NjRecord*)l.a.partials, (const unsigned long long*)l.a.cnt,
+                       l.a.blk_cb, l.a.blk_g0, (const int32_t*)l.a.pos_of_slot, l.a.ntest, l.a.nupd, l.a);
+}
+int njp_launch_scan(const NjpArgs& a, hipStream_t s)
+{
+    NjpScanLaunch l;
+    if (int rc = njp_prepare_scan(a, &l)) return rc;
+    njp_fire(l, s);
+    DPR_HIP(hipGetLastError());
+    return DPR_OK;
+}
+int njp_launch_post(const NjpArgs& a0, int64_t N, bool post2, hipStream_t s)
+{
+    NjpPostLaunch l;
+    njp_prepare_post(a0, N, post2, &l);
+    if (l.grid == 0u) return DPR_OK;
+    njp_fire(l, s);
     DPR_HIP(hipGetLastError());
     return DPR_OK;
 }
@@ -1356,20 +1391,22 @@
     return DPR_OK;
 }
 
+static int njp_fetch(void* dst, const void* src, size_t bytes, hipStream_t s)
+{
+    DPR_HIP(hipMemcpyAsync(dst, src, bytes, hipMemcpyDeviceToHost, s));
+    DPR_HIP(hipStreamSynchronize(s));
+    return DPR_OK;
+}
 int njp_epoch_order(const double* dU, const int32_t* slot_of_pos, int64_t P, int64_t n, std::vector<int32_t>& perm, bool stream_idle, hipStream_t s)
 {
     std::vector<double> hU((size_t)P);
-    if (stream_idle) {
-        DPR_HIP(hipMemcpy(hU.data(), dU, sizeof(double) * (size_t)P, hipMemcpyDeviceToHost));
-    } else {
-        DPR_HIP(hipMemcpyAsync(hU.data(), dU, sizeof(double) * (size_t)P, hipMemcpyDeviceToHost, s));
-        DPR_HIP(hipStreamSynchronize(s));
-    }
+    (void)stream_idle;
+    if (int rc = njp_fetch(hU.data(), dU, sizeof(double) * (size_t)P, s)) return rc;
     perm.clear();
     perm.reserve((size_t)n);
     if (slot_of_pos) {
         std::vector<int32_t> hslot((size_t)P);
-        DPR_HIP(hipMemcpy(hslot.data(), slot_of_pos, sizeof(int32_t) * (size_t)P, hipMemcpyDeviceToHost));
+        if (int rc = njp_fetch(hslot.data(), slot_of_pos, sizeof(int32_t) * (size_t)P, s)) return rc;
         for (int64_t p = 0; p < P; ++p)
             if (hslot[(size_t)p] >= 0) perm.push_back((int32_t)p);
     } else {
@@ -1413,6 +1450,8 @@
     const int g = e ? std::atoi(e) : 512;
     q.scan_grid = g < 1 ? 1 : (g > 1024 ? 1024 : g);
     if (const char* gi = std::getenv("DPR_NJ_GRAPH_ITERS")) { const int v = std::atoi(gi); if (v >= 1 && v <= 4096) q.graph_iters = v; }
+    if (const char* l = std::getenv("DPR_NJ_LEAD_FIRST")) { const long long v = std::atoll(l); if (v >= 0 && v <= (1 << 24)) q.lead_first = (int)v; }
+    if (const char* l = std::getenv("DPR_NJ_LEAD")) { const long long v = std::atoll(l); if (v >= 0 && v <= (1 << 24)) q.lead_next = (int)v; }
 }
 
 int njp_build(NjBuffers& b, hipStream_t s)
@@ -1457,7 +1496,7 @@
         tprev = t;
     };
     NjState st;
-    DPR_HIP(hipMemcpy(&st, b.st, sizeof(NjState), hipMemcpyDeviceToHost));
+    if (int rc = njp_fetch(&st, b.st, sizeof(NjState), s)) return rc;
     const int64_t n = st.n;
     if (st.status != 0 || n < 3) return DPR_OK;
     const double* Ucur = njp_current_u(q, st.it);
@@ -1492,7 +1531,7 @@
 {
     NjPruned& q = b.pr;
     NjState st;
-    DPR_HIP(hipMemcpy(&st, b.st, sizeof(NjState), hipMemcpyDeviceToHost));
+    if (int rc = njp_fetch(&st, b.st, sizeof(NjState), s)) return rc;
     const int64_t n = st.n;
     if (st.status != 0 || n < 3) return DPR_OK;
     if (q.graph) { (void)hipGraphExecDestroy(q.graph); q.graph = nullptr; }
@@ -1512,7 +1551,7 @@
     NjPruned& q = b.pr;
     NjState st;
     DPR_HIP(hipStreamSynchronize(s));
-    DPR_HIP(hipMemcpy(&st, b.st, sizeof(NjState), hipMemcpyDeviceToHost));
+    if (int rc = njp_fetch(&st, b.st, sizeof(NjState), s)) return rc;
     const int64_t n = st.n;
     if (st.status != 0 || n < 3) return DPR_OK;
     std::vector<int32_t> perm;
@@ -1631,9 +1670,13 @@
     return DPR_OK;
 }
 
+static std::atomic<bool> g_graph_instantiated{false};
+void njp_note_graph_instantiated() { g_graph_instantiated.store(true, std::memory_order_relaxed); }
+
 int njp_capture_graph(NjPruned& q, hipStream_t s, const std::function<int()>& enqueue)
 {
     const auto t0 = std::chrono::steady_clock::now();
+    const bool first = !g_graph_instantiated.load(std::memory_order_relaxed);
     ScopedGraph g;
     DPR_HIP(hipStreamBeginCapture(s, hipStreamCaptureModeThreadLocal));
     int rc = DPR_OK;
@@ -1643,10 +1686,37 @@
     if (e != hipSuccess) return hip_fail(e, "hipStreamEndCapture");
     e = hipGraphInstantiate(&q.graph, g, nullptr, nullptr, 0);
     if (e != hipSuccess) { q.graph = nullptr; return hip_fail(e, "hipGraphInstantiate"); }
+    njp_note_graph_instantiated();
     if (log_level("epoch") > 0)
-        std::fprintf(stderr, "[njp] graph capture + instantiate (P=%lld): %.2f ms\n", (long long)q.P,
+        std::fprintf(stderr, "[njp] graph capture + instantiate (P=%lld%s): %.2f ms\n", (long long)q.P, first ? ", first of the process" : "",
                      std::chrono::duration<double, std::milli>(std::chrono::steady_clock::now() - t0).count());
     return DPR_OK;
+}
+
+struct NjpIterationLaunch { NjpScanLaunch scan; NjpPostLaunch post; };
+static int njp_prepare_iteration(NjBuffers& b, NjpIterationLaunch* l)
+{
+    const NjpArgs a = njp_args(b, 0);
+    if (int rc = njp_prepare_scan(a, &l->scan)) return rc;
+    njp_prepare_post(a, b.N, njp_use_post2(b.pr), &l->post);
+    return DPR_OK;
+}
+static int njp_enqueue_stretch(const NjpIterationLaunch& l, int64_t count, hipStream_t s)
+{
+    for (int64_t k = 0; k < count; ++k) { njp_fire(l.scan, s); njp_fire(l.post, s); }
+    DPR_HIP(hipGetLastError());
+    return DPR_OK;
+}
+
+NjpSegmentPlan njp_segment_plan(int64_t seg, int64_t lead, int64_t graph_len)
+{
+    NjpSegmentPlan p;
+    if (seg <= 0) return p;
+    if (lead < 0) lead = 0;
+    p.head = lead < seg ? lead : seg;
+    if (graph_len >= 1) p.graphs = (seg - p.head) / graph_len;
+    p.tail = seg - p.head - p.graphs * (graph_len >= 1 ? graph_len : 0);
+    return p;
 }
 
 static int njp_run_segment(NjBuffers& b, int64_t it0, int64_t todo, hipStream_t s)
@@ -1670,14 +1740,32 @@
         q.fresh = false;
     }
     const bool timing = b.kt && b.kt->stride > 0 && q.sh_world <= 1;
-    const bool use_graph = q.sh_world <= 1 && todo >= q.graph_iters && !timing;
-    if (use_graph && !q.graph)
-        if (int rc = njp_capture_graph(q, s, [&] { return njp_enqueue_iteration(b, s); })) return rc;
-    int64_t done = 0;
-    if (use_graph)
-        for (; done + q.graph_iters <= todo; done += q.graph_iters) DPR_HIP(hipGraphLaunch(q.graph, s));
-    for (; done < todo; ++done)
-        if (int rc = njp_enqueue_iteration(b, s, timing && (it0 + done) % b.kt->stride == 0)) return rc;
+    if (q.sh_world > 1 || timing) {
+        for (int64_t done = 0; done < todo; ++done)
+            if (int rc = njp_enqueue_iteration(b, s, timing && (it0 + done) % b.kt->stride == 0)) return rc;
+        q.run_eager += todo;
+        return njp_launch_finish(njp_args(b, v0), s);
+    }
+    NjpIterationLaunch il;
+    if (int rc = njp_prepare_iteration(b, &il)) return rc;
+    const int64_t lead = q.graph ? 0 : g_graph_instantiated.load(std::memory_order_relaxed) ? q.lead_next : q.lead_first;
+    const NjpSegmentPlan plan = njp_segment_plan(todo, lead, q.graph_iters);
+    const bool tlog = log_level("epoch") >= 2 && plan.head > 0;
+    const auto t0 = std::chrono::steady_clock::now();
+    if (int rc = njp_enqueue_stretch(il, plan.head, s)) return rc;
+    if (tlog) {
+        const double us = std::chrono::duration<double, std::micro>(std::chrono::steady_clock::now() - t0).count();
+        std::fprintf(stderr, "[njp] eager head (P=%lld): %lld iterations enqueued in %.1f us, %.2f us per iteration\n", (long long)q.P,
+                     (long long)plan.head, us, us / (double)plan.head);
+    }
+    if (plan.graphs > 0 && !q.graph) {
+        if (int rc = njp_capture_graph(q, s, [&]() -> int { njp_fire(il.scan, s); njp_fire(il.post, s); DPR_HIP(hipGetLastError()); return DPR_OK; })) return rc;
+        if (q.run_graphs++ == 0) q.run_lead_seen = q.run_eager + plan.head;
+    }
+    for (int64_t g = 0; g < plan.graphs; ++g) DPR_HIP(hipGraphLaunch(q.graph, s));
+    if (int rc = njp_enqueue_stretch(il, plan.tail, s)) return rc;
+    q.run_eager += plan.head + plan.tail;
+    q.run_replayed += plan.graphs * q.graph_iters;
     return njp_launch_finish(njp_args(b, v0), s);
 }
 
@@ -1784,7 +1872,7 @@
             if (seg > chunk) seg = chunk;
             NjState st0;
             DPR_HIP(hipStreamSynchronize(s));
-            DPR_HIP(hipMemcpy(&st0, b.st, sizeof(NjState), hipMemcpyDeviceToHost));
+            if (int rc = njp_fetch(&st0, b.st, sizeof(NjState), s)) return rc;
             units0 = st0.units_scanned;
         }
         if (int rc = njp_run_segment(b, it, seg, s)) return rc;
@@ -1792,7 +1880,7 @@
         if (watch && left > 0) {
             NjState st1;
             DPR_HIP(hipStreamSynchronize(s));
-            DPR_HIP(hipMemcpy(&st1, b.st, sizeof(NjState), hipMemcpyDeviceToHost));
+            if (int rc = njp_fetch(&st1, b.st, sizeof(NjState), s)) return rc;
             if (st1.status != 0) continue;
             const double listed = (double)(st1.units_scanned - units0) - (first_of_epoch ? (double)q.utot : 0.0);
             const double iters = (double)seg - (first_of_epoch ? 1.0 : 0.0);
diff --git a/include/dipper_hip.h b/include/dipper_hip.h
--- a/include/dipper_hip.h
+++ b/include/dipper_hip.h
@@ -114,6 +114,8 @@
 int dpr_ctx_set_nj_multi_plan(dpr_ctx *ctx, int plan);
 int dpr_ctx_set_nj_adaptive(dpr_ctx *ctx, int on);
 int dpr_get_nj_adaptive_stats(dpr_ctx *ctx, int64_t *stream_iterations, int64_t *stream_epochs);
+int dpr_get_nj_graph_stats(dpr_ctx *ctx, int64_t *graphs, int64_t *replayed, int64_t *eager, int64_t *lead_seen);
+int dpr_njp_segment_plan(int64_t seg, int64_t lead, int64_t graph_len, int64_t *head, int64_t *graphs, int64_t *tail);
 int dpr_ctx_set_nj_exchange(dpr_ctx *ctx, int plan);
 int dpr_ctx_set_debug_fault(dpr_ctx *ctx, int64_t iteration, int rank);
 int dpr_get_nj_exchange_info(dpr_ctx *ctx, int *active_plan, int64_t *launches, int64_t *collectives, char *note, int cap);
```

Result: no change. 34650, median of 6 (+1.5%).
